# PAMRec/PAMRec

Measured on NVIDIA B200. Metric: train samples/sec, higher is better.
Workload: dtype f32

## Files before the change

pamrec_b200/csrc/api.cu:

```cuda
#include <cmath>
#include <cstdarg>
#include <cstdio>
#include <cstdlib>
#include <string>
#include <vector>

#include "comm.h"
#include "head2.h"
#include "kernels.h"
#include "layout.h"

using namespace pamrec;

struct Xchg {
  std::vector<int64_t> soff, scnt, roff, rcnt;
  int64_t n_send = 0, n_recv = 0;
};

struct PamrecHandle_ {
  PamrecConfig cfg;
  Layout L;
  PamrecBuffers buf;
  bool bound = false;
  int debug = 0;
  std::string err;
  int64_t launches = 0;
  Prof prof;
  BnSet bn[BN_COUNT];
  std::vector<int> h_seg_id, h_seg_tab;
  Comm comm;
  int* h_counts = nullptr;
  Xchg xc[3];
  bool xc_users = false;
  bool sharded() const { return cfg.table_mode == PAMREC_TABLES_SHARDED; }
  bool sibling() const { return cfg.model_kind != PAMREC_MODEL_PAMREC; }
  bool replicated() const { return cfg.table_mode == PAMREC_TABLES_REPLICATED && cfg.world_size > 1; }
  cudaStream_t side = nullptr;
  cudaEvent_t ev_side[16] = {};
  cudaEvent_t ev_join = nullptr, ev_plan = nullptr, ev_bucket = nullptr;
  int ev_next = 0;
  const void* plan_for = nullptr;
  int plan_rows = -1;
  void* mbox = nullptr;
  void* mbox_peer[kP2PMaxWorld] = {};
  bool mbox_open = false;
  unsigned* head_bar = nullptr;
  bool head_trace = false;
  unsigned long long* head_trace_cta = nullptr;
  uint32_t coop_epoch = 0;
  Head2 head2;
  int head2_grid = 0;
  bool use_head2() const { return head2_grid > 0 && (cfg.world_size == 1 || mbox_open); }
  uint32_t* mbox_err() const { return static_cast<uint32_t*>(mbox); }
  int64_t xr_dense() const { return (L.dense_numel + 63) / 64 * 64; }
  int64_t xr_floats() const { return xr_dense() + (replicated() ? sp2_rep_floats(cfg.n_items, cfg.n_cates, cfg.n_users) : 0); }
  char* xr_region(int p) const { return static_cast<char*>(mbox_peer[p]) + p2p_xr_offset(cfg.world_size); }
  bool use_xr() const { return mbox_open && cfg.world_size > 1; }
  uint32_t xr_epoch = 0;
  float* rep_grad_in() const { return use_xr() ? xr_xbuf(xr_region(cfg.rank)) + xr_dense() : wf("rep.grad"); }
  float* rep_grad_out() const {
    return use_xr() ? xr_xbuf(xr_region(cfg.rank)) + p2p_xr_cap(cfg.world_size, xr_floats()) + xr_dense() : wf("rep.grad");
  }
  ~PamrecHandle_() {
    if (h_counts) cudaFreeHost(h_counts);
    for (int p = 0; p < kP2PMaxWorld; ++p)
      if (mbox_peer[p] && mbox_peer[p] != mbox) cudaIpcCloseMemHandle(mbox_peer[p]);
    if (mbox) cudaFree(mbox);
    if (head_bar) cudaFree(head_bar);
    if (head_trace_cta) cudaFree(head_trace_cta);
    for (auto e : ev_side) if (e) cudaEventDestroy(e);
    if (ev_join) cudaEventDestroy(ev_join);
    if (ev_plan) cudaEventDestroy(ev_plan);
    if (ev_bucket) cudaEventDestroy(ev_bucket);
    if (side) cudaStreamDestroy(side);
  }
  template <typename F>
  void fork(cudaStream_t main, F fn) {
    cudaEvent_t e = ev_side[ev_next];
    ev_next = (ev_next + 1) % 16;
    cudaEventRecord(e, main);
    cudaStreamWaitEvent(side, e, 0);
    fn(side);
  }
  void join(cudaStream_t main) {
    cudaEventRecord(ev_join, side);
    cudaStreamWaitEvent(main, ev_join, 0);
  }

  float* P(int64_t off) const { return buf.dense_param + off; }
  float* G(int64_t off) const { return buf.dense_grad + off; }
  template <typename T>
  T* ws(const std::string& name) const { return reinterpret_cast<T*>(static_cast<char*>(buf.workspace) + L.ws_off(name)); }
  float* wf(const std::string& name) const { return ws<float>(name); }
  int* wi(const std::string& name) const { return ws<int>(name); }
  double* wd(const std::string& name) const { return ws<double>(name); }
};

struct ProfBind {
  PamrecHandle h; int64_t l0; Prof* prev;
  explicit ProfBind(PamrecHandle hh) : h(hh), l0(hh->prof.launches), prev(g_prof) { g_prof = &hh->prof; }
  ~ProfBind() { h->launches = h->prof.launches - l0; g_prof = prev; }
};

static int fail(PamrecHandle h, const char* fmt, ...) {
  char buf[512];
  va_list ap;
  va_start(ap, fmt);
  vsnprintf(buf, sizeof buf, fmt, ap);
  va_end(ap);
  if (h) h->err = buf;
  return -1;
}
static int check_cuda(PamrecHandle h, const char* where) {
  cudaError_t e = cudaGetLastError();
  if (e != cudaSuccess) return fail(h, "%s: %s", where, cudaGetErrorString(e));
  return 0;
}

extern "C" {

const char* pamrec_version(void) { return "pamrec_b200 0.1 (sm_100a)"; }

int pamrec_abi_sizes(int64_t out[6]) {
  if (!out) return -1;
  out[0] = sizeof(PamrecConfig); out[1] = sizeof(PamrecBatch); out[2] = sizeof(PamrecBuffers);
  out[3] = sizeof(PamrecTensorInfo); out[4] = sizeof(PamrecLines); out[5] = sizeof(PamrecVocab);
  return 0;
}

int pamrec_create(const PamrecConfig* cfg, PamrecHandle* out) {
  if (!cfg || !out) return -1;
  *out = nullptr;
  if (cfg->n_users < 1 || cfg->n_items < 1 || cfg->n_cates < 1) return -2;
  if (cfg->max_seq_len < 1 || cfg->max_seq_len > PAMREC_MAX_T) return -3;
  if (cfg->max_batch < 1) return -4;
  const int world = cfg->world_size < 1 ? 1 : cfg->world_size;
  if (world > 64 || cfg->rank < 0 || cfg->rank >= world) return -5;
  if (cfg->table_mode != PAMREC_TABLES_LOCAL && cfg->table_mode != PAMREC_TABLES_SHARDED && cfg->table_mode != PAMREC_TABLES_REPLICATED) return -6;
  if (world > 1 && cfg->table_mode == PAMREC_TABLES_LOCAL) return -6;
  if (cfg->table_mode != PAMREC_TABLES_SHARDED && (int64_t)cfg->n_items + cfg->n_cates + cfg->n_users >= ((int64_t)1 << 31)) return -7;
  if (cfg->loss_kind != PAMREC_LOSS_XENT && cfg->loss_kind != PAMREC_LOSS_SOFTMAX) return -8;
  if (cfg->loss_kind == PAMREC_LOSS_SOFTMAX) {
    const int g = cfg->softmax_group < 1 ? 1 : cfg->softmax_group;
    if (g > 1024 || (world > 1 && PAMREC_GROUP % g != 0)) return -8;
  }
  {
    int64_t big = cfg->n_items > cfg->n_users ? cfg->n_items : cfg->n_users;
    if (cfg->n_cates > big) big = cfg->n_cates;
    if (((big + world - 1) / world) * world >= ((int64_t)1 << 31)) return -7;
  }
  if (cfg->model_kind < PAMREC_MODEL_PAMREC || cfg->model_kind > PAMREC_MODEL_SASREC) return -9;
  if (cfg->model_kind != PAMREC_MODEL_PAMREC && (world != 1 || cfg->table_mode != PAMREC_TABLES_LOCAL || cfg->loss_kind != PAMREC_LOSS_XENT))
    return -9;
  const int di = cfg->item_dim ? cfg->item_dim : PAMREC_ITEM_DIM, dc = cfg->cate_dim ? cfg->cate_dim : PAMREC_CATE_DIM;
  const int du = cfg->user_dim ? cfg->user_dim : PAMREC_USER_DIM;
  if (!((di == 16 && dc == 4) || (di == 32 && dc == 8)) || !(du == 16 || du == 20 || du == 40)) return -10;
  if (cfg->model_kind == PAMREC_MODEL_PAMREC && (di != PAMREC_ITEM_DIM || dc != PAMREC_CATE_DIM || du != PAMREC_USER_DIM)) return -10;
  PamrecHandle h = new PamrecHandle_();
  h->cfg = *cfg;
  h->cfg.world_size = world;
  h->cfg.item_dim = di; h->cfg.cate_dim = dc; h->cfg.user_dim = du;
  if (h->cfg.softmax_group < 1) h->cfg.softmax_group = 1;
  h->L.build(h->cfg);
  const int n_seg = (int)h->L.dense.size();
  h->h_seg_id.assign((size_t)h->L.dense_numel, 0);
  h->h_seg_tab.assign((size_t)n_seg * 4, 0);
  for (int s = 0; s < n_seg; ++s) {
    const TensorDesc& t = h->L.dense[s];
    h->h_seg_tab[4 * s] = (int)t.offset;
    h->h_seg_tab[4 * s + 1] = (int)t.numel;
    h->h_seg_tab[4 * s + 2] = t.flags;
    for (int64_t i = 0; i < t.numel; ++i) h->h_seg_id[(size_t)(t.offset + i)] = s;
  }
  *out = h;
  return 0;
}

int pamrec_destroy(PamrecHandle h) {
  delete h;
  return 0;
}
const char* pamrec_last_error(PamrecHandle h) { return h ? h->err.c_str() : "null handle"; }
int64_t pamrec_dense_numel(PamrecHandle h) { return h ? h->L.dense_numel : -1; }
int64_t pamrec_bn_numel(PamrecHandle h) { return h ? h->L.bn_numel : -1; }
size_t pamrec_workspace_bytes(PamrecHandle h) { return h ? h->L.ws_bytes : 0; }
int64_t pamrec_last_launch_count(PamrecHandle h) { return h ? h->launches : -1; }
int64_t pamrec_shard_rows(PamrecHandle h, int64_t vocab_rows) { return h ? h->L.rows_of(vocab_rows) : -1; }

int pamrec_comm_unique_id(const char* nccl_path, char id_out[PAMREC_COMM_ID_BYTES]) {
  std::string err;
  if (Comm::unique_id(nccl_path, id_out, &err)) { fprintf(stderr, "pamrec_comm_unique_id: %s\n", err.c_str()); return -1; }
  return 0;
}
int pamrec_comm_init(PamrecHandle h, const char* nccl_path, const char id[PAMREC_COMM_ID_BYTES]) {
  if (!h || !id) return -1;
  if (h->comm.init(nccl_path, id, h->cfg.world_size, h->cfg.rank)) { h->err = "comm_init: " + h->comm.err; return -1; }
  return 0;
}
int pamrec_comm_mailbox_create(PamrecHandle h, char handle_out[PAMREC_IPC_HANDLE_BYTES]) {
  if (!h || !handle_out) return -1;
  static_assert(sizeof(cudaIpcMemHandle_t) == PAMREC_IPC_HANDLE_BYTES, "cudaIpcMemHandle_t is 64 bytes");
  if (h->cfg.world_size > kP2PMaxWorld) return fail(h, "mailboxes support at most %d ranks", kP2PMaxWorld);
  if (!h->mbox) {
    const size_t bytes = p2p_mailbox_bytes(h->cfg.world_size, h->xr_floats());
    if (cudaMalloc(&h->mbox, bytes) != cudaSuccess) return check_cuda(h, "mailbox alloc");
    cudaMemset(h->mbox, 0, bytes);
    cudaDeviceSynchronize();
  }
  cudaIpcMemHandle_t ih;
  if (cudaIpcGetMemHandle(&ih, h->mbox) != cudaSuccess) return check_cuda(h, "cudaIpcGetMemHandle");
  memcpy(handle_out, &ih, sizeof ih);
  return 0;
}
int pamrec_comm_mailbox_open(PamrecHandle h, const char* handles) {
  if (!h || !handles || !h->mbox) return -1;
  for (int p = 0; p < h->cfg.world_size; ++p) {
    if (p == h->cfg.rank) { h->mbox_peer[p] = h->mbox; continue; }
    cudaIpcMemHandle_t ih;
    memcpy(&ih, handles + (size_t)p * PAMREC_IPC_HANDLE_BYTES, sizeof ih);
    void* ptr = nullptr;
    if (cudaIpcOpenMemHandle(&ptr, ih, cudaIpcMemLazyEnablePeerAccess) != cudaSuccess) return check_cuda(h, "cudaIpcOpenMemHandle");
    h->mbox_peer[p] = ptr;
  }
  h->mbox_open = true;
  return 0;
}
int pamrec_comm_destroy(PamrecHandle h) {
  if (!h) return -1;
  h->comm.destroy();
  return 0;
}

static const std::vector<TensorDesc>* pool_of(PamrecHandle h, int pool) {
  if (!h) return nullptr;
  if (pool == PAMREC_POOL_DENSE) return &h->L.dense;
  if (pool == PAMREC_POOL_BN) return &h->L.bn;
  if (pool == PAMREC_POOL_WORKSPACE) return &h->L.ws;
  return nullptr;
}
int pamrec_tensor_count(PamrecHandle h, int pool) {
  auto* v = pool_of(h, pool);
  return v ? (int)v->size() : -1;
}
int pamrec_tensor_info(PamrecHandle h, int pool, int index, PamrecTensorInfo* out) {
  auto* v = pool_of(h, pool);
  if (!v || !out || index < 0 || index >= (int)v->size()) return -1;
  const TensorDesc& t = (*v)[index];
  memset(out, 0, sizeof *out);
  snprintf(out->name, sizeof out->name, "%s", t.name.c_str());
  out->pool = t.pool; out->dtype = t.dtype; out->flags = t.flags;
  out->offset = t.offset; out->numel = t.numel; out->ndim = t.ndim;
  for (int i = 0; i < 4; ++i) out->shape[i] = t.shape[i];
  return 0;
}

static BnSet make_bn(PamrecHandle h, int id, const char* name) {
  const BnOff& o = h->L.bnoff[id];
  BnSet s;
  s.C = o.C;
  s.gamma = h->P(o.gamma); s.beta = h->P(o.beta);
  s.dgamma = h->G(o.gamma); s.dbeta = h->G(o.beta);
  s.mmean = h->buf.bn_moving + o.mm; s.mvar = h->buf.bn_moving + o.mv;
  std::string p = std::string("bn.") + name;
  s.sums = h->wd(p + ".sums"); s.stat = h->wf(p + ".stat"); s.bsums = h->wd("bn.bsums") + h->L.bn_bsums_off[id];
  return s;
}

static int build_head(PamrecHandle h, cudaStream_t st);
static HeadDyn head_dyn(PamrecHandle h, const PamrecBatch* b, bool training, int slot0);

int pamrec_bind(PamrecHandle h, const PamrecBuffers* bufs, void* stream) {
  if (!h || !bufs) return -1;
  cudaStream_t st = (cudaStream_t)stream;
  if (bufs->workspace_bytes < h->L.ws_bytes) return fail(h, "workspace too small: %zu < %zu", bufs->workspace_bytes, h->L.ws_bytes);
  if (!bufs->dense_param || !bufs->dense_grad || !bufs->dense_m || !bufs->dense_v || !bufs->bn_moving || !bufs->item_w ||
      !bufs->cate_w || !bufs->ulong_w || !bufs->ushort_w || !bufs->workspace)
    return fail(h, "null buffer");
  int ndev = 0;
  if (cudaGetDeviceCount(&ndev) != cudaSuccess || ndev == 0) { cudaGetLastError(); return fail(h, "no CUDA device: the CUDA path is the only path"); }
  h->buf = *bufs;
  if (init_encoder_kernels(h->cfg.max_seq_len)) return check_cuda(h, "shared-memory opt-in of the encoder kernels");
  if (h->cfg.model_kind == PAMREC_MODEL_SASREC && init_sas_kernels(h->cfg.max_seq_len))
    return check_cuda(h, "shared-memory opt-in of the SASRec attention kernels");
  if (init_attn_mma_kernels(h->cfg.max_seq_len)) return check_cuda(h, "shared-memory opt-in of the MMA attention kernels");
  if (!h->side) {
    if (cudaStreamCreateWithFlags(&h->side, cudaStreamNonBlocking) != cudaSuccess) return fail(h, "cannot create the side stream");
    for (auto& e : h->ev_side) cudaEventCreateWithFlags(&e, cudaEventDisableTiming);
    cudaEventCreateWithFlags(&h->ev_join, cudaEventDisableTiming);
    cudaEventCreateWithFlags(&h->ev_plan, cudaEventDisableTiming);
    cudaEventCreateWithFlags(&h->ev_bucket, cudaEventDisableTiming);
  }
  static const char* names[BN_COUNT] = {"s0", "s1", "e0", "g0", "e1", "g1", "t0", "t1"};
  for (int i = 0; i < BN_COUNT; ++i) h->bn[i] = make_bn(h, i, names[i]);
  size_t need = sparse_temp_bytes(h->L.cub_keys);
  if (!h->sharded()) { const size_t n2 = sp2_temp_bytes(h->L.cub_keys); need = n2 > need ? n2 : need; }
  size_t have = (size_t)h->L.ws[h->L.ws_index["cub_temp"]].numel;
  if (need > have) return fail(h, "cub temp storage: need %zu have %zu", need, have);
  cudaMemsetAsync(h->buf.workspace, 0, h->L.ws_bytes, st);
  if (h->sharded() || h->sibling()) {
    cudaMemsetAsync(h->wi("sp.item.slot"), 0xFF, (size_t)h->L.rows_of(h->cfg.n_items) * 4, st);
    cudaMemsetAsync(h->wi("sp.cate.slot"), 0xFF, (size_t)h->L.rows_of(h->cfg.n_cates) * 4, st);
    if (h->cfg.model_kind != PAMREC_MODEL_SASREC)
      cudaMemsetAsync(h->wi("sp.user.slot"), 0xFF, (size_t)h->L.rows_of(h->cfg.n_users) * 4, st);
  } else {
    cudaMemsetAsync(h->wi("sp2.slot"), 0xFF, ((size_t)h->cfg.n_items + h->cfg.n_cates + h->cfg.n_users) * 4, st);
  }
  if (h->sharded() && !h->h_counts &&
      cudaMallocHost(&h->h_counts, sizeof(int) * (8 * (size_t)h->cfg.world_size + 4)) != cudaSuccess)
    return fail(h, "cudaMallocHost for the exchange counts failed");
  cudaMemcpyAsync(h->wi("seg_id"), h->h_seg_id.data(), h->h_seg_id.size() * 4, cudaMemcpyHostToDevice, st);
  cudaMemcpyAsync(h->wi("seg_tab"), h->h_seg_tab.data(), h->h_seg_tab.size() * 4, cudaMemcpyHostToDevice, st);
  if (h->sibling()) h->head2_grid = 0;
  else if (int rc = build_head(h, st)) return rc;
  cudaStreamSynchronize(st);
  h->bound = true;
  return check_cuda(h, "bind");
}

static int check_batch(PamrecHandle h, const PamrecBatch* b, bool training) {
  if (!h) return -1;
  if (!h->bound) return fail(h, "pamrec_bind has not been called");
  if (!b) return fail(h, "null batch");
  if (b->batch == 0 && (h->sharded() || h->cfg.world_size > 1)) return 0;
  if (b->batch < 1 || b->batch > h->cfg.max_batch) return fail(h, "batch %d outside [1, %d]", b->batch, h->cfg.max_batch);
  if (h->sibling()) {
    if (!b->satisfied_item_history || !b->satisfied_cate_history || !b->satisfied_mask || !b->item_history || !b->item_cate_history ||
        !b->mask || !b->items || !b->cates)
      return fail(h, "null batch field (the sibling models also read satisfied_item_history / satisfied_cate_history / satisfied_mask)");
    const bool sas = h->cfg.model_kind == PAMREC_MODEL_SASREC;
    if (training && (!b->labels_satisfied || (!sas && (!b->users || !b->labels_play)))) return fail(h, "null label field");
    return 0;
  }
  if (training && b->batch % PAMREC_GROUP != 0)
    return fail(h, "training batch %d is not a multiple of %d (pamrec.py:73-75)", b->batch, PAMREC_GROUP);
  if (training && h->cfg.loss_kind == PAMREC_LOSS_SOFTMAX && b->batch % h->cfg.softmax_group != 0)
    return fail(h, "training batch %d is not a multiple of the softmax group %d (base_model.py:224-225)", b->batch, h->cfg.softmax_group);
  if (!b->item_history || !b->item_cate_history || !b->item_loop_times_history || !b->mask || !b->items || !b->cates)
    return fail(h, "null batch field");
  if (training && (!b->users || !b->labels_satisfied || !b->labels_play || !b->plays)) return fail(h, "null label field");
  return 0;
}

static Sp2 make_sp2(PamrecHandle h, const PamrecBatch* b) {
  Sp2 s;
  memset(&s, 0, sizeof s);
  const PamrecConfig& c = h->cfg;
  s.item_hist = b->item_history; s.cate_hist = b->item_cate_history; s.items = b->items; s.cates = b->cates; s.users = b->users;
  s.B = b->batch; s.N = (int64_t)b->batch * c.max_seq_len;
  s.n_items = c.n_items; s.n_cates = c.n_cates; s.n_users = c.n_users;
  s.keys = h->wi("sp2.keys"); s.idx = h->wi("sp2.idx"); s.skeys = h->wi("sp2.skeys"); s.sidx = h->wi("sp2.sidx"); s.uidx = h->wi("sp2.uidx");
  s.ukeys[0] = h->wi("sp.item.ukeys"); s.ukeys[1] = h->wi("sp.cate.ukeys"); s.ukeys[2] = h->wi("sp.user.ukeys");
  s.nuniq = h->wi("sp.nuniq"); s.meta = h->wi("sp2.meta");
  s.accum[0] = h->wf("sp.item.accum"); s.accum[1] = h->wf("sp.cate.accum");
  s.dflag[0] = h->wi("sp2.dflag"); s.dflag[1] = s.dflag[0] + h->L.cub_keys_table;
  s.l2sq = h->wd("sp2.l2sq"); s.undedup = h->wd("sp_normsq");
  s.w[0] = h->buf.item_w; s.m[0] = h->buf.item_m; s.v[0] = h->buf.item_v;
  s.w[1] = h->buf.cate_w; s.m[1] = h->buf.cate_m; s.v[1] = h->buf.cate_v;
  s.w[2] = h->buf.ulong_w; s.m[2] = h->buf.ulong_m; s.v[2] = h->buf.ulong_v;
  s.w[3] = h->buf.ushort_w; s.m[3] = h->buf.ushort_m; s.v[3] = h->buf.ushort_v;
  s.dX0 = h->wf("g_a"); s.dT = h->wf("d_tgt_total");
  if (h->replicated()) { s.mode = SP2_DENSE; s.rep_grad = h->rep_grad_in(); }
  else if (c.sparse_adam_mode == PAMREC_ADAM_LAZY) s.mode = SP2_FUSED;
  else { s.mode = SP2_COMPACT; s.slot = h->wi("sp2.slot"); }
  return s;
}
static AdamP make_adam(PamrecHandle h, float lr_t) {
  const PamrecConfig& c = h->cfg;
  AdamP a;
  a.lr = lr_t; a.b1 = c.beta1; a.b2 = c.beta2; a.eps = c.epsilon; a.l2 = c.embed_l2; a.clip = c.max_grad_norm; a.is_clip = c.is_clip_norm;
  a.lr_dev = nullptr;
  return a;
}

static const char* const kShardName[3] = {"item", "cate", "user"};
static const ShardDim& shard_dim(PamrecHandle h, int t) { return t == 0 ? h->L.sh_item : (t == 1 ? h->L.sh_cate : h->L.sh_user); }

static SparseTable req_table(PamrecHandle h, int t) {
  SparseTable s;
  memset(&s, 0, sizeof s);
  const ShardDim& d = shard_dim(h, t);
  std::string p = std::string("sp.") + kShardName[t] + ".";
  s.keys = h->wi(p + "keys"); s.idx = h->wi(p + "idx"); s.skeys = h->wi(p + "skeys"); s.sidx = h->wi(p + "sidx");
  s.uidx = h->wi(p + "uidx"); s.ukeys = h->wi(p + "ukeys");
  s.width = d.width; s.n_rows = d.rps * h->cfg.world_size;
  s.accum = d.width ? h->wf(p + "accum") : nullptr;
  s.nuniq = h->wi("sp.nuniq") + t;
  s.normsq = h->wd("sp_normsq") + t;
  return s;
}
static SparseTable own_table(PamrecHandle h, int t, bool user_short = false) {
  SparseTable s;
  memset(&s, 0, sizeof s);
  const ShardDim& d = shard_dim(h, t);
  std::string q = std::string("so.") + kShardName[t] + ".";
  s.keys = h->wi(q + "keys"); s.idx = h->wi(q + "idx"); s.skeys = h->wi(q + "skeys"); s.sidx = h->wi(q + "sidx");
  s.uidx = h->wi(q + "uidx"); s.ukeys = h->wi(q + "ukeys");
  s.slot = h->wi(std::string("sp.") + kShardName[t] + ".slot");
  s.n_rows = d.rps;
  s.nuniq = h->wi("sp.nuniq") + 4 + t;
  double* ns = h->wd("sp_normsq");
  if (t == 0) { s.width = kI; s.w = h->buf.item_w; s.m = h->buf.item_m; s.v = h->buf.item_v; s.accum = h->wf(q + "accum"); s.normsq = ns; }
  else if (t == 1) { s.width = kC; s.w = h->buf.cate_w; s.m = h->buf.cate_m; s.v = h->buf.cate_v; s.accum = h->wf(q + "accum"); s.normsq = ns + 1; }
  else if (!user_short) { s.width = PAMREC_USER_DIM; s.w = h->buf.ulong_w; s.m = h->buf.ulong_m; s.v = h->buf.ulong_v; s.normsq = ns + 2; }
  else { s.width = PAMREC_USER_DIM; s.w = h->buf.ushort_w; s.m = h->buf.ushort_m; s.v = h->buf.ushort_v; s.normsq = ns + 3; }
  return s;
}

static int shard_exchange_fwd(PamrecHandle h, const PamrecBatch* b, bool training, cudaStream_t st) {
  const int W = h->cfg.world_size, B = b->batch, T = h->cfg.max_seq_len;
  const int64_t N = (int64_t)B * T;
  void* tmp = h->ws<char>("cub_temp");
  const size_t tmp_bytes = (size_t)h->L.ws[h->L.ws_index.at("cub_temp")].numel;
  int* cs = h->wi("sh.counts_send");
  int* cr = h->wi("sh.counts_recv");
  cudaMemsetAsync(cs, 0, sizeof(int) * 4 * W, st);
  const int nt = training ? 3 : 2;
  h->xc_users = training;
  for (int t = 0; t < nt; ++t) {
    const ShardDim& d = shard_dim(h, t);
    SparseTable req = req_table(h, t);
    const int* hist = t == 0 ? b->item_history : (t == 1 ? b->item_cate_history : b->users);
    const int* tgt = t == 0 ? b->items : (t == 1 ? b->cates : nullptr);
    const int64_t n_hist = t < 2 ? N : B, n_tgt = t < 2 ? B : 0;
    if (launch_sparse_plan(req, hist, tgt, n_hist, n_tgt, W, d.rps, d.rps * W, false, tmp, tmp_bytes, st))
      return fail(h, "cub sort failed");
    std::string p = std::string("sh.") + kShardName[t] + ".";
    launch_shard_route(req, n_hist + n_tgt, W, d.rps, h->wi(p + "off"), cs, t, h->wi(p + "send_ids"), h->wi(p + "inv"), st);
  }
  {
    PAMREC_PROF("xchg_counts", 1, st);
    if (h->comm.all_to_all(cs, cr, 4, COMM_I32, st)) return fail(h, "nccl: %s", h->comm.err.c_str());
    cudaMemcpyAsync(h->h_counts, cs, sizeof(int) * 4 * W, cudaMemcpyDeviceToHost, st);
    cudaMemcpyAsync(h->h_counts + 4 * W, cr, sizeof(int) * 4 * W, cudaMemcpyDeviceToHost, st);
    h->h_counts[8 * W] = 0;
    if (h->mbox_open) cudaMemcpyAsync(h->h_counts + 8 * W, h->mbox_err(), sizeof(int), cudaMemcpyDeviceToHost, st);
    if (cudaStreamSynchronize(st) != cudaSuccess) return check_cuda(h, "exchange counts");
    if (h->h_counts[8 * W]) return fail(h, "peer mailbox all-reduce timed out at sync point %d (a rank left the step?)", h->h_counts[8 * W] - 1);
  }
  for (int t = 0; t < 3; ++t) {
    Xchg& x = h->xc[t];
    x.soff.assign(W, 0); x.scnt.assign(W, 0); x.roff.assign(W, 0); x.rcnt.assign(W, 0);
    int64_t so = 0, ro = 0;
    for (int p = 0; p < W; ++p) {
      x.scnt[p] = t < nt ? h->h_counts[4 * p + t] : 0;
      x.rcnt[p] = t < nt ? h->h_counts[4 * W + 4 * p + t] : 0;
      x.soff[p] = so; so += x.scnt[p];
      x.roff[p] = ro; ro += x.rcnt[p];
    }
    x.n_send = so; x.n_recv = ro;
    if (ro > shard_dim(h, t).cap_recv) return fail(h, "exchange overflow on table %s: %lld rows", kShardName[t], (long long)ro);
  }
  {
    PAMREC_PROF("xchg_ids", 1, st);
    int xrc = h->comm.group_start();
    for (int t = 0; t < nt && !xrc; ++t) {
      const Xchg& x = h->xc[t];
      std::string p = std::string("sh.") + kShardName[t] + ".";
      xrc |= h->comm.all_to_all_v(h->wi(p + "send_ids"), x.soff.data(), x.scnt.data(), h->wi(p + "recv_ids"), x.roff.data(),
                                  x.rcnt.data(), 1, COMM_I32, st);
    }
    xrc |= h->comm.group_end();
    if (xrc) return fail(h, "nccl: %s", h->comm.err.c_str());
  }
  if (training) {
    int prc = 0;
    h->fork(st, [&](cudaStream_t s2) {
      for (int t = 0; t < 3; ++t) {
        SparseTable own = own_table(h, t);
        std::string p = std::string("sh.") + kShardName[t] + ".";
        prc |= launch_sparse_plan(own, h->wi(p + "recv_ids"), nullptr, h->xc[t].n_recv, 0, 1, 0, own.n_rows, true, tmp, tmp_bytes, s2);
      }
      cudaEventRecord(h->ev_plan, s2);
    });
    if (prc) return fail(h, "cub sort failed");
  }
  launch_serve_rows(h->buf.item_w, h->wi("sh.item.recv_ids"), h->xc[0].n_recv, kI, h->wf("sh.item.xrows"), st);
  launch_serve_rows(h->buf.cate_w, h->wi("sh.cate.recv_ids"), h->xc[1].n_recv, kC, h->wf("sh.cate.xrows"), st);
  {
    PAMREC_PROF("xchg_rows", 1, st);
    int xrc = h->comm.group_start();
    for (int t = 0; t < 2 && !xrc; ++t) {
      const Xchg& x = h->xc[t];
      std::string p = std::string("sh.") + kShardName[t] + ".";
      xrc |= h->comm.all_to_all_v(h->wf(p + "xrows"), x.roff.data(), x.rcnt.data(), h->wf(p + "rows"), x.soff.data(),
                                  x.scnt.data(), shard_dim(h, t).width, COMM_F32, st);
    }
    xrc |= h->comm.group_end();
    if (xrc) return fail(h, "nccl: %s", h->comm.err.c_str());
  }
  return 0;
}

static int embed_forward(PamrecHandle h, const PamrecBatch* b, bool training, float* x0, cudaStream_t st) {
  const int B = b->batch, T = h->cfg.max_seq_len;
  if (!h->sharded()) {
    launch_embed_fwd(b->item_history, b->item_cate_history, b->items, b->cates, h->buf.item_w, h->buf.cate_w, h->P(h->L.pos), x0,
                     h->wf("tgt"), B, T, st);
    return 0;
  }
  if (int rc = shard_exchange_fwd(h, b, training, st)) return rc;
  const int64_t N = (int64_t)B * T;
  const int* ii = h->wi("sh.item.inv");
  const int* ci = h->wi("sh.cate.inv");
  launch_embed_fwd(ii, ci, ii + N, ci + N, h->wf("sh.item.rows"), h->wf("sh.cate.rows"), h->P(h->L.pos), x0, h->wf("tgt"), B, T, st);
  return 0;
}

int pamrec_gather_fwd(PamrecHandle h, const PamrecBatch* b, float* x0_out, void* stream) {
  if (int rc = check_batch(h, b, false)) return rc;
  if (h->sibling()) return fail(h, "pamrec_gather_fwd is PAMRec's fused gather; the sibling models gather inside pamrec_forward");
  ProfBind _pb(h);
  cudaStream_t st = (cudaStream_t)stream;
  if (int rc = embed_forward(h, b, false, x0_out ? x0_out : h->wf("x0"), st)) return rc;
  return check_cuda(h, "gather_fwd");
}

static DenseP dense_p(const float* X, int ldx, int M, int groups, int K, int N, const float* W, int ws, const float* bias,
                      int bs, float* Z, int ldz) {
  DenseP p;
  memset(&p, 0, sizeof p);
  p.X = X; p.ldx = ldx; p.M = M; p.n_groups = groups; p.K = K; p.N = N;
  p.W = W; p.w_stride = ws; p.bias = bias; p.b_stride = bs; p.Z = Z; p.ldz = ldz;
  return p;
}
static void set_in_bn(DenseP& p, const BnSet& s) { p.in_stat = s.stat; p.in_gamma = s.gamma; p.in_beta = s.beta; }
static void set_in_bn_dw(DenseDwP& p, const BnSet& s) { p.in_stat = s.stat; p.in_gamma = s.gamma; p.in_beta = s.beta; }

static int sib_forward(PamrecHandle h, const PamrecBatch* b, int training, float* pred_out, cudaStream_t st);
static int sib_backward(PamrecHandle h, const PamrecBatch* b, cudaStream_t st);
static int sib_apply(PamrecHandle h, const PamrecBatch* b, int64_t step, cudaStream_t st);
static int sas_forward(PamrecHandle h, const PamrecBatch* b, int training, float* pred_out, cudaStream_t st);
static int sas_backward(PamrecHandle h, const PamrecBatch* b, cudaStream_t st);
static int head_forward(PamrecHandle h, const PamrecBatch* b, bool training, float* pred_out, cudaStream_t st);

int pamrec_forward(PamrecHandle h, const PamrecBatch* b, int training, float* pred_out, void* stream) {
  if (int rc = check_batch(h, b, training != 0)) return rc;
  ProfBind _pb(h);
  cudaStream_t st = (cudaStream_t)stream;
  if (h->cfg.model_kind == PAMREC_MODEL_SASREC) return sas_forward(h, b, training, pred_out, st);
  if (h->sibling()) return sib_forward(h, b, training, pred_out, st);
  const Layout& L = h->L;
  const int B = b->batch, T = h->cfg.max_seq_len, N = B * T;
  float* x0 = h->wf("x0");
  int* ctl = h->wi("bucket_ctl");
  const bool bucket_aside = !h->sharded();
  if (bucket_aside) {
    h->fork(st, [&](cudaStream_t s2) {
      launch_bucket_plan(b->item_loop_times_history, N, h->wi("bucket"), h->wi("perm"), ctl, h->wi("tile_bucket"), h->wi("tile_begin"),
                         h->wi("tile_count"), s2);
      cudaEventRecord(h->ev_bucket, s2);
    });
  }
  if (int rc = embed_forward(h, b, training != 0, x0, st)) return rc;
  if (training && !h->sharded() && B > 0) {
    int prc = 0;
    h->fork(st, [&](cudaStream_t s2) {
      prc |= launch_sp2_plan(make_sp2(h, b), h->ws<char>("cub_temp"), (size_t)L.ws[L.ws_index.at("cub_temp")].numel, s2);
      cudaEventRecord(h->ev_plan, s2);
    });
    if (prc) return fail(h, "cub sort failed");
    h->plan_for = b->item_history; h->plan_rows = B;
  }
  if (bucket_aside) cudaStreamWaitEvent(st, h->ev_bucket, 0);
  else launch_bucket_plan(b->item_loop_times_history, N, h->wi("bucket"), h->wi("perm"), ctl, h->wi("tile_bucket"),
                          h->wi("tile_begin"), h->wi("tile_count"), st);
  const int max_tiles = N / kTokTile + kNB + 1;
  const float* xin = x0;
  for (int k = 0; k < 2; ++k) {
    const BlockOff& o = L.blk[k];
    std::string p = "blk" + std::to_string(k) + ".";
    launch_proj_fwd(xin, h->wi("perm"), ctl, h->wi("tile_bucket"), h->wi("tile_begin"), h->wi("tile_count"), max_tiles,
                    h->P(o.wq), h->P(o.wk), h->P(o.wv), h->P(o.ln_a_beta), h->P(o.ln_a_gamma), h->wf(p + "qin"), h->wf(p + "Q"),
                    h->wf(p + "K"), h->wf(p + "V"), st);
    if (T <= 128)
      launch_attn_fwd_mma(h->wf(p + "Q"), h->wf(p + "K"), h->wf(p + "V"), h->wf(p + "qin"), b->mask, h->wf(p + "y"), h->wf(p + "pv"), h->wf(p + "ml"), B, T, st);
    else
      launch_attn_fwd(h->wf(p + "Q"), h->wf(p + "K"), h->wf(p + "V"), h->wf(p + "qin"), b->mask, h->wf(p + "y"), h->wf(p + "pv"), h->wf(p + "ml"), B, T, st);
    float* hdbg = (training && (h->debug & PAMREC_DEBUG_SAVE_FFN_HIDDEN)) ? h->wf(k == 0 ? "d_Q" : "d_K") : nullptr;
    launch_ffn_fwd(h->wf(p + "y"), h->P(o.w1), h->P(o.b1), h->P(o.w2), h->P(o.b2), h->P(o.ln_b_beta), h->P(o.ln_b_gamma),
                   h->wf(p + "out"), hdbg, N, st);
    xin = h->wf(p + "out");
  }
  if (h->use_head2()) {
    HeadDyn d = head_dyn(h, b, training != 0, 0);
    d.pred = pred_out;
    if (launch_head2_fwd(h->head2, d, h->head2_grid, training ? "head_fwd" : "head_score", st)) return check_cuda(h, "cooperative head launch");
  } else if (int rc = head_forward(h, b, training != 0, pred_out, st)) {
    return rc;
  }
  return check_cuda(h, "forward");
}

static int head_forward(PamrecHandle h, const PamrecBatch* b, bool training, float* pred_out, cudaStream_t st) {
  const Layout& L = h->L;
  const int B = b->batch, T = h->cfg.max_seq_len, N = B * T;
  const int W = h->cfg.world_size;
  const int Bg = b->global_batch > 0 ? b->global_batch : B * W;
  const double cntN = (double)Bg * T, cntB = (double)Bg;
  int crc = 0;
  auto sync_finalize = [&](std::initializer_list<int> ids, double cnt, bool with_scalars) {
    if (!training) return;
    if (W > 1 && !crc) {
      PAMREC_PROF("allreduce_bn_fwd", 1, st);
      crc |= h->comm.group_start();
      for (int id : ids) crc |= h->comm.all_reduce(h->bn[id].sums, 2 * (int64_t)h->bn[id].C, COMM_F64, st);
      if (with_scalars) crc |= h->comm.all_reduce(h->wd("dp.scalars"), 8, COMM_F64, st);
      crc |= h->comm.group_end();
    }
    for (int id : ids) launch_bn_finalize(h->bn[id], cnt, st);
  };
  if (training && W > 1) {
    cudaMemsetAsync(h->wd("dp.scalars"), 0, 8 * sizeof(double), st);
    launch_count_valid_groups(b->plays, B, h->wd("dp.scalars"), st);
  }
  const float* H = h->wf("blk1.out");
  BnSet* bn = h->bn;
  if (!training) {
    for (int i = 0; i < BN_COUNT; ++i) launch_bn_eval_stat(bn[i], st);
  }
  {
    DenseP p = dense_p(H, kD, N, 1, kD, 20, h->P(L.score.w0), 0, h->P(L.score.b0), 0, h->wf("z1"), 20);
    p.out_sums = training ? bn[BN_S0].sums : nullptr;
    launch_dense_fwd(p, st);
    sync_finalize({BN_S0}, cntN, true);
    DenseP q = dense_p(h->wf("z1"), 20, N, 1, 20, 1, h->P(L.score.w1), 0, h->P(L.score.b1), 0, h->wf("z2"), 1);
    set_in_bn(q, bn[BN_S0]);
    q.out_sums = training ? bn[BN_S1].sums : nullptr;
    launch_dense_fwd(q, st);
    sync_finalize({BN_S1}, cntN, false);
  }
  launch_pool_fwd(H, h->wf("z2"), bn[BN_S1], b->mask, h->wf("new_long"), B, T, st);
  {
    DenseP e0 = dense_p(h->wf("new_long"), kD, B, 5, kD, 100, h->P(L.expert.w0), 4000, h->P(L.expert.b0), 100, h->wf("ze0"), 500);
    for (int g = 0; g < 5; ++g) { e0.x_off[g] = 0; e0.z_off[g] = g * 100; }
    e0.out_sums = training ? bn[BN_E0].sums : nullptr;
    launch_dense_fwd(e0, st);
    DenseP g0 = dense_p(h->wf("new_long"), kD, B, 2, kD, 64, h->P(L.gate.w0), 2560, h->P(L.gate.b0), 64, h->wf("zg0"), 128);
    for (int g = 0; g < 2; ++g) { g0.x_off[g] = 0; g0.z_off[g] = g * 64; }
    g0.out_sums = training ? bn[BN_G0].sums : nullptr;
    launch_dense_fwd(g0, st);
    sync_finalize({BN_E0, BN_G0}, cntB, false);
    DenseP e1 = dense_p(h->wf("ze0"), 500, B, 5, 100, 64, h->P(L.expert.w1), 6400, h->P(L.expert.b1), 64, h->wf("ze1"), 320);
    for (int g = 0; g < 5; ++g) { e1.x_off[g] = g * 100; e1.z_off[g] = g * 64; }
    set_in_bn(e1, bn[BN_E0]);
    e1.out_sums = training ? bn[BN_E1].sums : nullptr;
    launch_dense_fwd(e1, st);
    DenseP g1 = dense_p(h->wf("zg0"), 128, B, 2, 64, 5, h->P(L.gate.w1), 320, h->P(L.gate.b1), 5, h->wf("zg1"), 10);
    for (int g = 0; g < 2; ++g) { g1.x_off[g] = g * 64; g1.z_off[g] = g * 5; }
    set_in_bn(g1, bn[BN_G0]);
    g1.out_sums = training ? bn[BN_G1].sums : nullptr;
    launch_dense_fwd(g1, st);
    sync_finalize({BN_E1, BN_G1}, cntB, false);
  }
  launch_combine_fwd(h->wf("ze1"), h->wf("zg1"), bn[BN_E1], bn[BN_G1], h->wf("tgt"), h->wf("u"), B, st);
  {
    DenseP t0 = dense_p(h->wf("u"), 168, B, 3, 84, 100, h->P(L.tower.w0), 8400, h->P(L.tower.b0), 100, h->wf("zt0"), 300);
    t0.x_off[0] = 0; t0.x_off[1] = 84; t0.x_off[2] = 0;
    for (int g = 0; g < 3; ++g) t0.z_off[g] = g * 100;
    t0.out_sums = training ? bn[BN_T0].sums : nullptr;
    launch_dense_fwd(t0, st);
    sync_finalize({BN_T0}, cntB, false);
    DenseP t1 = dense_p(h->wf("zt0"), 300, B, 3, 100, 64, h->P(L.tower.w1), 6400, h->P(L.tower.b1), 64, h->wf("zt1"), 192);
    for (int g = 0; g < 3; ++g) { t1.x_off[g] = g * 100; t1.z_off[g] = g * 64; }
    set_in_bn(t1, bn[BN_T0]);
    t1.out_sums = training ? bn[BN_T1].sums : nullptr;
    launch_dense_fwd(t1, st);
    sync_finalize({BN_T1}, cntB, false);
    DenseP to = dense_p(h->wf("zt1"), 192, B, 3, 64, 1, h->P(L.tower.wout), 64, h->P(L.tower.bout), 1, h->wf("logits"), 3);
    for (int g = 0; g < 3; ++g) { to.x_off[g] = g * 64; to.z_off[g] = g; }
    set_in_bn(to, bn[BN_T1]);
    launch_dense_fwd(to, st);
  }
  if (pred_out) launch_sigmoid_col0(h->wf("logits"), pred_out, B, st);
  if (crc) return fail(h, "nccl: %s", h->comm.err.c_str());
  return 0;
}

static DenseDwP dw_p(const float* X, int ldx, int M, int groups, int K, int N, const float* dZ, int lddz, float* dW, int ws,
                     float* db, int bs) {
  DenseDwP p;
  memset(&p, 0, sizeof p);
  p.X = X; p.ldx = ldx; p.M = M; p.n_groups = groups; p.K = K; p.N = N; p.dZ = dZ; p.lddz = lddz;
  p.dW = dW; p.w_stride = ws; p.db = db; p.b_stride = bs;
  return p;
}
static DenseDxP dx_p(const float* dZ, int lddz, int M, int K, const float* Wbase, float* dX, int lddx, int accumulate) {
  DenseDxP p;
  memset(&p, 0, sizeof p);
  p.dZ = dZ; p.lddz = lddz; p.M = M; p.K = K; p.Wbase = Wbase; p.dX = dX; p.lddx = lddx; p.accumulate = accumulate;
  return p;
}
static void dx_add(DenseDxP& p, int slice, int out_off, int dz_off, int64_t w_off, int N) {
  if (slice >= p.n_slices) { p.n_slices = slice + 1; p.out_off[slice] = out_off; p.n_contrib[slice] = 0; }
  int c = p.n_contrib[slice]++;
  p.dz_off[slice][c] = dz_off; p.w_off[slice][c] = w_off; p.Ncon[slice][c] = N;
}

static HeadDyn head_dyn(PamrecHandle h, const PamrecBatch* b, bool training, int slot0) {
  HeadDyn d;
  memset(&d, 0, sizeof d);
  const int W = h->cfg.world_size;
  d.B = b->batch; d.T = h->cfg.max_seq_len; d.training = training ? 1 : 0; d.world = W; d.rank = h->cfg.rank;
  d.Bg = b->global_batch > 0 ? b->global_batch : b->batch * W;
  d.cntN = (double)d.Bg * d.T; d.cntB = (double)d.Bg;
  d.mask = b->mask; d.y_sat = b->labels_satisfied; d.y_play = b->labels_play; d.plays = b->plays;
  d.fuzhu_w = h->cfg.fuzhu_weight; d.order_w = h->cfg.order_weight;
  d.sm_group = h->cfg.loss_kind == PAMREC_LOSS_SOFTMAX ? h->cfg.softmax_group : 0;
  d.bar = h->head_bar;
  d.trace = h->head_trace ? reinterpret_cast<unsigned long long*>(h->head_bar + 64) + (slot0 ? 32 : 0) : nullptr;
  d.trace_cta = (h->head_trace && h->head_trace_cta) ? h->head_trace_cta + (slot0 ? 16 * 256 : 0) : nullptr;
  if (W > 1) {
    for (int p = 0; p < W; ++p) d.peer_ll[p] = reinterpret_cast<uint4*>(static_cast<char*>(h->mbox_peer[p]) + p2p_ll_offset());
    d.p2p_epoch = ++h->coop_epoch; d.p2p_slot0 = slot0; d.p2p_err = h->mbox_err();
  }
  return d;
}

static int build_head(PamrecHandle h, cudaStream_t st) {
  h->head2_grid = 0;
  if (getenv("PAMREC_HEAD_LEGACY") != nullptr) return 0;
  if (h->cfg.world_size > kP2PMaxWorld) return 0;
  const Layout& L = h->L;
  Head2& H = h->head2;
  memset(&H, 0, sizeof H);
  H.H = h->wf("blk1.out"); H.tgt = h->wf("tgt");
  H.s_w0 = h->P(L.score.w0); H.s_b0 = h->P(L.score.b0); H.s_w1 = h->P(L.score.w1); H.s_b1 = h->P(L.score.b1);
  H.e_w0 = h->P(L.expert.w0); H.e_b0 = h->P(L.expert.b0); H.e_w1 = h->P(L.expert.w1); H.e_b1 = h->P(L.expert.b1);
  H.g_w0 = h->P(L.gate.w0); H.g_b0 = h->P(L.gate.b0); H.g_w1 = h->P(L.gate.w1); H.g_b1 = h->P(L.gate.b1);
  H.t_w0 = h->P(L.tower.w0); H.t_b0 = h->P(L.tower.b0); H.t_w1 = h->P(L.tower.w1); H.t_b1 = h->P(L.tower.b1);
  H.t_wo = h->P(L.tower.wout); H.t_bo = h->P(L.tower.bout);
  H.ds_w0 = h->G(L.score.w0); H.ds_b0 = h->G(L.score.b0); H.ds_w1 = h->G(L.score.w1); H.ds_b1 = h->G(L.score.b1);
  H.de_w0 = h->G(L.expert.w0); H.de_b0 = h->G(L.expert.b0); H.de_w1 = h->G(L.expert.w1); H.de_b1 = h->G(L.expert.b1);
  H.dg_w0 = h->G(L.gate.w0); H.dg_b0 = h->G(L.gate.b0); H.dg_w1 = h->G(L.gate.w1); H.dg_b1 = h->G(L.gate.b1);
  H.dt_w0 = h->G(L.tower.w0); H.dt_b0 = h->G(L.tower.b0); H.dt_w1 = h->G(L.tower.w1); H.dt_b1 = h->G(L.tower.b1);
  H.dt_wo = h->G(L.tower.wout); H.dt_bo = h->G(L.tower.bout);
  H.wT = h->wf("head.wT");
  static_assert(kHead2Groups == 8, "layout.h: bn.gsums / bn.gbsums hold 8 copies");
  for (int i = 0; i < BN_COUNT; ++i) {
    H.bn[i] = h->bn[i];
    H.gsums[i] = h->wd("bn.gsums") + (size_t)kHead2Groups * L.bn_bsums_off[i];
    H.gbsums[i] = h->wd("bn.gbsums") + (size_t)kHead2Groups * L.bn_bsums_off[i];
  }
  H.z1 = h->wf("z1"); H.z2 = h->wf("z2"); H.aw = h->wf("pool.aw"); H.new_long = h->wf("new_long");
  H.ze0 = h->wf("ze0"); H.zg0 = h->wf("zg0"); H.ze1 = h->wf("ze1"); H.zg1 = h->wf("zg1"); H.u = h->wf("u");
  H.zt0 = h->wf("zt0"); H.zt1 = h->wf("zt1"); H.logits = h->wf("logits");
  H.d_logits = h->wf("d_logits"); H.d_t1 = h->wf("d_t1"); H.d_t0 = h->wf("d_t0"); H.d_e1 = h->wf("d_e1"); H.d_g1 = h->wf("d_g1");
  H.d_e0 = h->wf("d_e0"); H.d_g0 = h->wf("d_g0"); H.d_new_long = h->wf("d_new_long"); H.d_tgt = h->wf("d_tgt");
  H.d_z2 = h->wf("d_z2"); H.g_a = h->wf("g_a");
  H.loss_acc = h->wd("loss_acc"); H.dp_scalars = h->wd("dp.scalars");
  const int g2 = head2_grid();
  if (g2 <= 0) { cudaGetLastError(); return 0; }
  if (!h->head_bar) {
    if (cudaMalloc(&h->head_bar, 256 + 2 * 32 * 8) != cudaSuccess) return check_cuda(h, "head barrier alloc");
    cudaMemsetAsync(h->head_bar, 0, 256 + 2 * 32 * 8, st);
  }
  h->head2_grid = g2;
  return check_cuda(h, "head2");
}

static int head_backward(PamrecHandle h, const PamrecBatch* b, cudaStream_t st) {
  const Layout& L = h->L;
  const int B = b->batch, T = h->cfg.max_seq_len, N = B * T;
  const int W = h->cfg.world_size;
  const int Bg = b->global_batch > 0 ? b->global_batch : B * W;
  const double cntN = (double)Bg * T, cntB = (double)Bg;
  const float gs = 1.0f / (float)W;
  BnSet* bn = h->bn;
  int crc = 0;
  const float* Pb = h->buf.dense_param;
  launch_loss(h->wf("logits"), b->labels_satisfied, b->labels_play, b->plays, h->wf("d_logits"), h->wd("loss_acc"), B, Bg,
              W > 1 ? h->wd("dp.scalars") : nullptr, h->cfg.fuzhu_weight, h->cfg.order_weight,
              h->cfg.loss_kind == PAMREC_LOSS_SOFTMAX ? h->cfg.softmax_group : 0, st);
  cudaMemsetAsync(h->wd("bn.bsums"), 0, (size_t)L.ws[L.ws_index.at("bn.bsums")].numel * sizeof(double), st);
  auto sync_bsums = [&](std::initializer_list<int> ids) {
    if (W == 1 || crc) return;
    PAMREC_PROF("allreduce_bn_bwd", 1, st);
    crc |= h->comm.group_start();
    for (int id : ids) crc |= h->comm.all_reduce(bn[id].bsums, 2 * (int64_t)bn[id].C, COMM_F64, st);
    crc |= h->comm.group_end();
  };
  auto grad_of = [&](int id, const float* Z, double cnt) {
    BnGrad g; g.Z = Z; g.stat = bn[id].stat; g.gamma = bn[id].gamma; g.beta = bn[id].beta; g.bsums = bn[id].bsums; g.count = cnt;
    return g;
  };
  auto out_of = [&](int id, const float* Z) {
    BnGradOut o; o.Z = Z; o.stat = bn[id].stat; o.gamma = bn[id].gamma; o.beta = bn[id].beta; o.bsums = bn[id].bsums;
    return o;
  };
  auto dw_bn = [&](DenseDwP& w, int id, const float* Z, double cnt) {
    w.g = grad_of(id, Z, cnt); w.g_dgamma = bn[id].dgamma; w.g_dbeta = bn[id].dbeta; w.g_C = bn[id].C; w.g_scale = gs;
  };
  {
    DenseDwP w = dw_p(h->wf("zt1"), 192, B, 3, 64, 1, h->wf("d_logits"), 3, h->G(L.tower.wout), 64, h->G(L.tower.bout), 1);
    for (int g = 0; g < 3; ++g) { w.x_off[g] = g * 64; w.z_off[g] = g; }
    set_in_bn_dw(w, bn[BN_T1]);
    h->fork(st, [&](cudaStream_t s2) { launch_dense_dw(w, s2); });
    DenseDxP x = dx_p(h->wf("d_logits"), 3, B, 64, Pb, h->wf("d_t1"), 192, 0);
    for (int g = 0; g < 3; ++g) dx_add(x, g, g * 64, g, L.tower.wout + g * 64, 1);
    x.o = out_of(BN_T1, h->wf("zt1"));
    launch_dense_dx(x, st);
    sync_bsums({BN_T1});
    DenseDwP w1 = dw_p(h->wf("zt0"), 300, B, 3, 100, 64, h->wf("d_t1"), 192, h->G(L.tower.w1), 6400, h->G(L.tower.b1), 64);
    for (int g = 0; g < 3; ++g) { w1.x_off[g] = g * 100; w1.z_off[g] = g * 64; }
    set_in_bn_dw(w1, bn[BN_T0]);
    dw_bn(w1, BN_T1, h->wf("zt1"), cntB);
    h->fork(st, [&](cudaStream_t s2) { launch_dense_dw(w1, s2); });
    DenseDxP x1 = dx_p(h->wf("d_t1"), 192, B, 100, Pb, h->wf("d_t0"), 300, 0);
    for (int g = 0; g < 3; ++g) dx_add(x1, g, g * 100, g * 64, L.tower.w1 + (int64_t)g * 6400, 64);
    x1.g = grad_of(BN_T1, h->wf("zt1"), cntB);
    x1.o = out_of(BN_T0, h->wf("zt0"));
    launch_dense_dx(x1, st);
    sync_bsums({BN_T0});
    DenseDwP w0 = dw_p(h->wf("u"), 168, B, 3, 84, 100, h->wf("d_t0"), 300, h->G(L.tower.w0), 8400, h->G(L.tower.b0), 100);
    w0.x_off[0] = 0; w0.x_off[1] = 84; w0.x_off[2] = 0;
    for (int g = 0; g < 3; ++g) w0.z_off[g] = g * 100;
    dw_bn(w0, BN_T0, h->wf("zt0"), cntB);
    h->fork(st, [&](cudaStream_t s2) { launch_dense_dw(w0, s2); });
    DenseDxP x0 = dx_p(h->wf("d_t0"), 300, B, 84, Pb, h->wf("d_u"), 168, 0);
    dx_add(x0, 0, 0, 0, L.tower.w0, 100);
    dx_add(x0, 0, 0, 200, L.tower.w0 + 2 * 8400, 100);
    dx_add(x0, 1, 84, 100, L.tower.w0 + 8400, 100);
    x0.g = grad_of(BN_T0, h->wf("zt0"), cntB);
    launch_dense_dx(x0, st);
  }
  launch_combine_bwd(h->wf("ze1"), h->wf("zg1"), bn[BN_E1], bn[BN_G1], h->wf("d_u"), h->wf("d_e1"), h->wf("d_g1"),
                     h->wf("d_tgt"), B, st);
  {
    launch_bn_bwd_stats(bn[BN_E1], h->wf("d_e1"), h->wf("ze1"), B, st);
    launch_bn_bwd_stats(bn[BN_G1], h->wf("d_g1"), h->wf("zg1"), B, st);
    sync_bsums({BN_E1, BN_G1});
    DenseDwP we = dw_p(h->wf("ze0"), 500, B, 5, 100, 64, h->wf("d_e1"), 320, h->G(L.expert.w1), 6400, h->G(L.expert.b1), 64);
    for (int g = 0; g < 5; ++g) { we.x_off[g] = g * 100; we.z_off[g] = g * 64; }
    set_in_bn_dw(we, bn[BN_E0]);
    dw_bn(we, BN_E1, h->wf("ze1"), cntB);
    h->fork(st, [&](cudaStream_t s2) { launch_dense_dw(we, s2); });
    DenseDxP xe = dx_p(h->wf("d_e1"), 320, B, 100, Pb, h->wf("d_e0"), 500, 0);
    for (int g = 0; g < 5; ++g) dx_add(xe, g, g * 100, g * 64, L.expert.w1 + (int64_t)g * 6400, 64);
    xe.g = grad_of(BN_E1, h->wf("ze1"), cntB);
    xe.o = out_of(BN_E0, h->wf("ze0"));
    launch_dense_dx(xe, st);
    DenseDwP wg = dw_p(h->wf("zg0"), 128, B, 2, 64, 5, h->wf("d_g1"), 10, h->G(L.gate.w1), 320, h->G(L.gate.b1), 5);
    for (int g = 0; g < 2; ++g) { wg.x_off[g] = g * 64; wg.z_off[g] = g * 5; }
    set_in_bn_dw(wg, bn[BN_G0]);
    dw_bn(wg, BN_G1, h->wf("zg1"), cntB);
    h->fork(st, [&](cudaStream_t s2) { launch_dense_dw(wg, s2); });
    DenseDxP xg = dx_p(h->wf("d_g1"), 10, B, 64, Pb, h->wf("d_g0"), 128, 0);
    for (int g = 0; g < 2; ++g) dx_add(xg, g, g * 64, g * 5, L.gate.w1 + (int64_t)g * 320, 5);
    xg.g = grad_of(BN_G1, h->wf("zg1"), cntB);
    xg.o = out_of(BN_G0, h->wf("zg0"));
    launch_dense_dx(xg, st);
    sync_bsums({BN_E0, BN_G0});
    DenseDwP we0 = dw_p(h->wf("new_long"), kD, B, 5, kD, 100, h->wf("d_e0"), 500, h->G(L.expert.w0), 4000, h->G(L.expert.b0), 100);
    for (int g = 0; g < 5; ++g) { we0.x_off[g] = 0; we0.z_off[g] = g * 100; }
    dw_bn(we0, BN_E0, h->wf("ze0"), cntB);
    h->fork(st, [&](cudaStream_t s2) { launch_dense_dw(we0, s2); });
    DenseDwP wg0 = dw_p(h->wf("new_long"), kD, B, 2, kD, 64, h->wf("d_g0"), 128, h->G(L.gate.w0), 2560, h->G(L.gate.b0), 64);
    for (int g = 0; g < 2; ++g) { wg0.x_off[g] = 0; wg0.z_off[g] = g * 64; }
    dw_bn(wg0, BN_G0, h->wf("zg0"), cntB);
    h->fork(st, [&](cudaStream_t s2) { launch_dense_dw(wg0, s2); });
    DenseDxP xe0 = dx_p(h->wf("d_e0"), 500, B, kD, Pb, h->wf("d_new_long"), kD, 0);
    for (int g = 0; g < 5; ++g) dx_add(xe0, 0, 0, g * 100, L.expert.w0 + (int64_t)g * 4000, 100);
    xe0.g = grad_of(BN_E0, h->wf("ze0"), cntB);
    launch_dense_dx(xe0, st);
    DenseDxP xg0 = dx_p(h->wf("d_g0"), 128, B, kD, Pb, h->wf("d_new_long"), kD, 1);
    for (int g = 0; g < 2; ++g) dx_add(xg0, 0, 0, g * 64, L.gate.w0 + (int64_t)g * 2560, 64);
    xg0.g = grad_of(BN_G0, h->wf("zg0"), cntB);
    launch_dense_dx(xg0, st);
  }
  const float* H = h->wf("blk1.out");
  float* g_a = h->wf("g_a");
  launch_pool_bwd(H, h->wf("z2"), bn[BN_S1], b->mask, h->wf("d_new_long"), h->wf("d_z2"), g_a, B, T, st);
  launch_bn_bwd_stats(bn[BN_S1], h->wf("d_z2"), h->wf("z2"), N, st);
  sync_bsums({BN_S1});
  DenseDwP w1 = dw_p(h->wf("z1"), 20, N, 1, 20, 1, h->wf("d_z2"), 1, h->G(L.score.w1), 0, h->G(L.score.b1), 0);
  set_in_bn_dw(w1, bn[BN_S0]);
  dw_bn(w1, BN_S1, h->wf("z2"), cntN);
  h->fork(st, [&](cudaStream_t s2) { launch_dense_dw(w1, s2); });
  DenseDxP x1 = dx_p(h->wf("d_z2"), 1, N, 20, Pb, h->wf("d_a1"), 20, 0);
  dx_add(x1, 0, 0, 0, L.score.w1, 1);
  x1.g = grad_of(BN_S1, h->wf("z2"), cntN);
  x1.o = out_of(BN_S0, h->wf("z1"));
  launch_dense_dx(x1, st);
  sync_bsums({BN_S0});
  DenseDwP w0 = dw_p(H, kD, N, 1, kD, 20, h->wf("d_a1"), 20, h->G(L.score.w0), 0, h->G(L.score.b0), 0);
  dw_bn(w0, BN_S0, h->wf("z1"), cntN);
  h->fork(st, [&](cudaStream_t s2) { launch_dense_dw(w0, s2); });
  DenseDxP x0 = dx_p(h->wf("d_a1"), 20, N, kD, Pb, g_a, kD, 1);
  dx_add(x0, 0, 0, 0, L.score.w0, 20);
  x0.g = grad_of(BN_S0, h->wf("z1"), cntN);
  launch_dense_dx(x0, st);
  return crc;
}

int pamrec_backward(PamrecHandle h, const PamrecBatch* b, void* stream) {
  if (int rc = check_batch(h, b, true)) return rc;
  ProfBind _pb(h);
  cudaStream_t st = (cudaStream_t)stream;
  if (h->cfg.model_kind == PAMREC_MODEL_SASREC) return sas_backward(h, b, st);
  if (h->sibling()) return sib_backward(h, b, st);
  const Layout& L = h->L;
  const int B = b->batch, T = h->cfg.max_seq_len, N = B * T;
  int crc = 0;
  cudaMemsetAsync(h->buf.dense_grad, 0, (size_t)L.dense_numel * 4, st);
  cudaMemsetAsync(h->wd("loss_acc"), 0, 8 * sizeof(double), st);
  cudaMemsetAsync(h->wd("sp_normsq"), 0, 8 * sizeof(double), st);
  if (h->use_head2()) {
    cudaMemsetAsync(h->wd("bn.bsums"), 0, (size_t)L.ws[L.ws_index.at("bn.bsums")].numel * sizeof(double), st);
    HeadDyn d = head_dyn(h, b, true, 12);
    if (launch_head2_bwd(h->head2, d, h->head2_grid, st)) return check_cuda(h, "cooperative head launch");
    h->fork(st, [&](cudaStream_t s2) { launch_head2_dw(h->head2, B, s2); });
  } else {
    crc = head_backward(h, b, st);
  }
  float* g_a = h->wf("g_a");
  float* g_b = h->wf("g_b");
  const int max_tiles = N / kTokTile + kNB + 1;
  int* ctl = h->wi("bucket_ctl");
  for (int k = 1; k >= 0; --k) {
    const BlockOff& o = L.blk[k];
    std::string p = "blk" + std::to_string(k) + ".";
    const float* xin = k == 0 ? h->wf("x0") : h->wf("blk0.out");
    float* gout = k == 1 ? g_a : g_b;
    float* gin = k == 1 ? g_b : g_a;
    float* dQ = h->wf(k == 1 ? "blk1.d_Q" : "d_Q");
    float* dK = h->wf(k == 1 ? "blk1.d_K" : "d_K");
    float* dV = h->wf(k == 1 ? "blk1.d_V" : "d_V");
    float* dout = k == 1 ? h->wf("blk1.d_out") : gout;
    EncDwArgs dw{h->wf(p + "qin"), xin, dQ, dK, dV, h->wi("perm"), ctl, h->wf(p + "y"), h->P(o.ln_b_beta), h->P(o.ln_b_gamma),
                 h->wf(p + "h"), h->wf(p + "dhr"), dout, h->G(o.wq), h->G(o.wk), h->G(o.wv), h->G(o.w1), h->G(o.b1), h->G(o.w2),
                 h->G(o.b2), N, true};
    launch_ffn_bwd(h->wf(p + "y"), gout, h->P(o.w1), h->P(o.b1), h->P(o.w2), h->P(o.ln_b_beta), h->P(o.ln_b_gamma), h->wf("d_y"),
                   h->wf(p + "h"), h->wf(p + "dhr"), k == 1 ? dout : nullptr, h->G(o.ln_b_beta), h->G(o.ln_b_gamma), N, st);
    h->fork(st, [&](cudaStream_t s2) { launch_enc_dw(dw, s2); });
    if (T <= 128)
      launch_attn_bwd_mma(h->wf(p + "Q"), h->wf(p + "K"), h->wf(p + "V"), h->wf("d_y"), h->wf(p + "pv"), h->wf(p + "ml"),
                          b->mask, dQ, dK, dV, B, T, st);
    else
      launch_attn_bwd(h->wf(p + "Q"), h->wf(p + "K"), h->wf(p + "V"), h->wf("d_y"), h->wf(p + "pv"), h->wf(p + "ml"),
                      b->mask, dQ, dK, dV, B, T, st);
    dw.ffn = false;
    h->fork(st, [&](cudaStream_t s2) { launch_enc_dw(dw, s2); });
    launch_proj_bwd(xin, h->wf("d_y"), dQ, dK, dV, h->wi("perm"), ctl, h->wi("tile_bucket"), h->wi("tile_begin"), h->wi("tile_count"),
                    max_tiles, h->P(o.wq), h->P(o.wk), h->P(o.wv), h->P(o.ln_a_beta), h->P(o.ln_a_gamma), gin, h->G(o.ln_a_beta),
                    h->G(o.ln_a_gamma), st);
  }
  launch_embed_bwd_reduce(g_a, h->wf("d_tgt"), h->wf("d_tgt_total"), h->G(L.pos), h->wd("sp_normsq") + 4,
                          h->sharded() ? nullptr : h->wd("sp_normsq"), B, T, st);
  h->join(st);
  if (crc) return fail(h, "nccl: %s", h->comm.err.c_str());
  return check_cuda(h, "backward");
}

static void peer_allreduce_grads(PamrecHandle h, cudaStream_t st) {
  XrArgs a;
  memset(&a, 0, sizeof a);
  const int W = h->cfg.world_size;
  for (int p = 0; p < W; ++p) a.peer[p] = h->xr_region(p);
  a.world = W; a.rank = h->cfg.rank; a.epoch = ++h->xr_epoch;
  a.cap = p2p_xr_cap(W, h->xr_floats());
  a.dense_grad = h->buf.dense_grad; a.n_dense = h->L.dense_numel;
  a.scalars[0] = h->wd("sp_normsq"); a.n_scalars[0] = 8;
  a.scalars[1] = h->wd("loss_acc"); a.n_scalars[1] = 4;
  a.counter = reinterpret_cast<unsigned*>(h->xr_region(h->cfg.rank) + 128);
  a.err = h->mbox_err();
  launch_xr_allreduce(a, h->buf.dense_grad, st);
}

int pamrec_apply_gradients(PamrecHandle h, const PamrecBatch* b, int64_t step, void* stream) {
  if (int rc = check_batch(h, b, true)) return rc;
  ProfBind _pb(h);
  if (h->sibling()) return sib_apply(h, b, step, (cudaStream_t)stream);
  if (step < 0) return fail(h, "step must be >= 1 (or 0: advance the device step counter)");
  if (step == 0 && (h->sharded() || h->cfg.world_size > 1)) return fail(h, "the device step counter (step = 0) needs one GPU with whole tables");
  cudaStream_t st = (cudaStream_t)stream;
  const Layout& L = h->L;
  const PamrecConfig& c = h->cfg;
  const int B = b->batch, T = c.max_seq_len;
  const int64_t N = (int64_t)B * T;
  const double b1 = c.beta1, b2 = c.beta2;
  const double tstep = step > 0 ? (double)step : 1.0;
  const float lr_t = (float)((double)c.learning_rate * std::sqrt(1.0 - std::pow(b2, tstep)) / (1.0 - std::pow(b1, tstep)));
  const float* lr_dev = nullptr;
  if (!h->sharded()) {
    launch_adam_step(step, h->wd("adam.step"), c.learning_rate, c.beta1, c.beta2, h->wf("adam.lr"), st);
    lr_dev = h->wf("adam.lr");
  }
  double* reg = h->wd("loss_acc") + 3;
  void* tmp = h->ws<char>("cub_temp");
  size_t tmp_bytes = (size_t)L.ws[L.ws_index.at("cub_temp")].numel;
  bool dense_aside = false;
  const float* dX0 = h->wf("g_a");
  const float* dT = h->wf("d_tgt_total");
  if (h->sharded()) {
    Comm& cm = h->comm;
    int crc = 0;
    if (!h->xc_users) return fail(h, "apply_gradients needs pamrec_forward(training=1) on the same batch");
    for (int t = 0; t < 2; ++t) {
      SparseTable req = req_table(h, t);
      const int col = t == 0 ? 0 : kI;
      launch_sparse_segreduce(req, N + B, N, dX0, kD, col, dT, kE, col, req.normsq, st);
    }
    {
      PAMREC_PROF("xchg_grads", 1, st);
      crc |= cm.group_start();
      for (int t = 0; t < 2; ++t) {
        const Xchg& x = h->xc[t];
        std::string p = std::string("sh.") + kShardName[t] + ".";
        crc |= cm.all_to_all_v(req_table(h, t).accum, x.soff.data(), x.scnt.data(), h->wf(p + "xrows"), x.roff.data(), x.rcnt.data(),
                               shard_dim(h, t).width, COMM_F32, st);
      }
      crc |= cm.group_end();
    }
    cudaStreamWaitEvent(st, h->ev_plan, 0);
    for (int t = 0; t < 3; ++t) {
      SparseTable own = own_table(h, t);
      const int64_t nr = h->xc[t].n_recv;
      std::string p = std::string("sh.") + kShardName[t] + ".";
      if (t < 2) launch_sparse_segreduce(own, nr, nr, h->wf(p + "xrows"), own.width, 0, nullptr, 0, 0, h->wd("sh.scratch"), st);
      launch_sparse_l2norm(own, nr, c.embed_l2, reg, st);
      if (t == 2) launch_sparse_l2norm(own_table(h, 2, true), nr, c.embed_l2, reg, st);
    }
    if (h->use_xr()) {
      peer_allreduce_grads(h, st);
    } else {
      PAMREC_PROF("allreduce_grads", 1, st);
      crc |= cm.group_start();
      crc |= cm.all_reduce(h->buf.dense_grad, L.dense_numel, COMM_F32, st);
      crc |= cm.all_reduce(h->wd("sp_normsq"), 8, COMM_F64, st);
      crc |= cm.all_reduce(h->wd("loss_acc"), 4, COMM_F64, st);
      crc |= cm.group_end();
    }
    if (crc) return fail(h, "nccl: %s", cm.err.c_str());
    for (int t = 0; t < 3; ++t) {
      SparseTable own = own_table(h, t);
      const int64_t nr = h->xc[t].n_recv;
      launch_sparse_adam(own, nr, c.sparse_adam_mode, c.embed_l2, lr_t, c.beta1, c.beta2, c.epsilon, c.max_grad_norm, c.is_clip_norm, st);
      if (t == 2)
        launch_sparse_adam(own_table(h, 2, true), nr, c.sparse_adam_mode, c.embed_l2, lr_t, c.beta1, c.beta2, c.epsilon,
                           c.max_grad_norm, c.is_clip_norm, st);
      launch_slot_reset(own, nr, st);
    }
  } else {
    if (c.world_size == 1) {
      dense_aside = true;
      h->fork(st, [&](cudaStream_t s2) {
        launch_dense_norm(h->buf.dense_param, h->buf.dense_grad, h->wi("seg_tab"), (int)L.dense.size(), c.layer_l2, h->wd("seg_normsq"),
                          h->wd("sp_normsq") + 4, reg, s2);
        launch_dense_adam(h->buf.dense_param, h->buf.dense_grad, h->buf.dense_m, h->buf.dense_v, h->wi("seg_id"), h->wi("seg_tab"),
                          h->wd("seg_normsq"), L.dense_numel, c.layer_l2, lr_t, lr_dev, c.beta1, c.beta2, c.epsilon, c.max_grad_norm,
                          c.is_clip_norm, s2);
      });
    }
    const bool planned = h->plan_for == b->item_history && h->plan_rows == B;
    h->plan_for = nullptr;
    const Sp2 s2 = make_sp2(h, b);
    AdamP ap = make_adam(h, lr_t);
    ap.lr_dev = lr_dev;
    if (planned) cudaStreamWaitEvent(st, h->ev_plan, 0);
    else if (launch_sp2_plan(s2, tmp, tmp_bytes, st)) return fail(h, "cub sort failed");
    launch_sp2_walk(s2, ap, st);
   
    if (h->replicated()) {
      Sp2 s3 = s2;
      if (h->use_xr()) {
        peer_allreduce_grads(h, st);
        s3.rep_grad = h->rep_grad_out();
      } else {
        Comm& cm = h->comm;
        int crc = 0;
        {
          PAMREC_PROF("allreduce_grads", 1, st);
          crc |= cm.group_start();
          crc |= cm.all_reduce(h->buf.dense_grad, L.dense_numel, COMM_F32, st);
          crc |= cm.all_reduce(s2.rep_grad, sp2_rep_floats(c.n_items, c.n_cates, c.n_users), COMM_F32, st);
          crc |= cm.all_reduce(h->wd("sp_normsq"), 8, COMM_F64, st);
          crc |= cm.all_reduce(h->wd("loss_acc"), 4, COMM_F64, st);
          crc |= cm.group_end();
        }
        if (crc) return fail(h, "nccl: %s", cm.err.c_str());
      }
      launch_sp2_rep_l2(s3, st);
      launch_sp2_adam_sweep(s3, ap, c.sparse_adam_mode == PAMREC_ADAM_LAZY ? 1 : 0, st);
     
    } else if (s2.mode == SP2_FUSED) {
      launch_sp2_lazy_finish(s2, ap, st);
    } else {
      launch_sp2_adam_sweep(s2, ap, 0, st);
    }
  }
  const int n_seg = (int)L.dense.size();
  if (dense_aside) {
    h->join(st);
  } else {
    launch_dense_norm(h->buf.dense_param, h->buf.dense_grad, h->wi("seg_tab"), n_seg, c.layer_l2, h->wd("seg_normsq"),
                      h->wd("sp_normsq") + 4, reg, st);
    launch_dense_adam(h->buf.dense_param, h->buf.dense_grad, h->buf.dense_m, h->buf.dense_v, h->wi("seg_id"), h->wi("seg_tab"),
                      h->wd("seg_normsq"), L.dense_numel, c.layer_l2, lr_t, lr_dev, c.beta1, c.beta2, c.epsilon, c.max_grad_norm,
                      c.is_clip_norm, st);
  }
  launch_finish_losses(h->wd("loss_acc"), h->wf("losses"), h->sharded() ? nullptr : h->wd("sp2.l2sq"), c.embed_l2, h->wd("sp_normsq"), st);
 
  return check_cuda(h, "apply_gradients");
}

#include "api_sibling.inl"

int pamrec_train_step(PamrecHandle h, const PamrecBatch* b, int64_t step, float* losses_out, void* stream) {
  if (!h) return -1;
  const int64_t l0 = h->prof.launches;
  if (int rc = pamrec_forward(h, b, 1, nullptr, stream)) return rc;
  if (int rc = pamrec_backward(h, b, stream)) return rc;
  if (int rc = pamrec_apply_gradients(h, b, step, stream)) return rc;
  if (losses_out)
    cudaMemcpyAsync(losses_out, h->wf("losses"), 5 * sizeof(float), cudaMemcpyDeviceToDevice, (cudaStream_t)stream);
  h->launches = h->prof.launches - l0;
  return check_cuda(h, "train_step");
}

int pamrec_comm_all_reduce(PamrecHandle h, void* dptr, int64_t count, int dtype, void* stream) {
  if (!h) return -1;
  CommType t = dtype == PAMREC_F64 ? COMM_F64 : (dtype == PAMREC_I32 ? COMM_I32 : COMM_F32);
  if (h->comm.all_reduce(dptr, count, t, (cudaStream_t)stream)) return fail(h, "nccl: %s", h->comm.err.c_str());
  return 0;
}

int pamrec_bench_gather(PamrecHandle h, const int32_t* item_ids, const int32_t* cate_ids, const int32_t* tgt_items,
                        const int32_t* tgt_cates, int64_t n_rows, int32_t T, float* out, void* stream) {
  if (!h || !h->bound) return fail(h, "not bound");
  if (h->sibling()) return fail(h, "bench_gather measures PAMRec's fused gather");
  if (T < 1 || T > h->cfg.max_seq_len) return fail(h, "T outside the position table");
  ProfBind _pb(h);
  launch_embed_fwd(item_ids, cate_ids, tgt_items, tgt_cates, h->buf.item_w, h->buf.cate_w, h->P(h->L.pos), out, nullptr, n_rows,
                   T, (cudaStream_t)stream);
  return check_cuda(h, "bench_gather");
}

int pamrec_bench_table_adam(PamrecHandle h, int64_t step, void* stream) {
  if (!h || !h->bound) return fail(h, "not bound");
  ProfBind _pb(h);
  const PamrecConfig& c = h->cfg;
  const double b1 = c.beta1, b2 = c.beta2;
  const float lr_t = (float)((double)c.learning_rate * std::sqrt(1.0 - std::pow(b2, (double)step)) / (1.0 - std::pow(b1, (double)step)));
  if (h->sharded() || h->sibling()) return fail(h, "bench_table_adam runs on PAMRec's whole tables");
  PamrecBatch nb;
  memset(&nb, 0, sizeof nb);
  Sp2 s2 = make_sp2(h, &nb);
  s2.mode = SP2_COMPACT; s2.slot = h->wi("sp2.slot");
  launch_sp2_adam_sweep(s2, make_adam(h, lr_t), 0, (cudaStream_t)stream);
  return check_cuda(h, "bench_table_adam");
}

int pamrec_set_debug(PamrecHandle h, int flags) {
  if (!h) return -1;
  h->debug = flags;
  h->head_trace = (flags & PAMREC_DEBUG_HEAD_TRACE) != 0;
  if (h->head_trace && !h->head_trace_cta && cudaMalloc(&h->head_trace_cta, 2 * 16 * 256 * 8) == cudaSuccess)
    cudaMemset(h->head_trace_cta, 0, 2 * 16 * 256 * 8);
  return 0;
}
int pamrec_head_trace_ctas(PamrecHandle h, int backward, uint64_t* out ) {
  if (!h || !out || !h->head_trace_cta) return -1;
  cudaDeviceSynchronize();
  if (cudaMemcpy(out, h->head_trace_cta + (backward ? 16 * 256 : 0), 16 * 256 * 8, cudaMemcpyDeviceToHost) != cudaSuccess) return check_cuda(h, "head trace");
  return 0;
}
int pamrec_head_trace(PamrecHandle h, int backward, uint64_t out[32]) {
  if (!h || !out || !h->head_bar) return -1;
  cudaDeviceSynchronize();
  if (cudaMemcpy(out, reinterpret_cast<unsigned long long*>(h->head_bar + 64) + (backward ? 32 : 0), 32 * 8, cudaMemcpyDeviceToHost) != cudaSuccess)
    return check_cuda(h, "head trace");
  return 0;
}
int pamrec_profile_enable(PamrecHandle h, int on) {
  if (!h) return -1;
  h->prof.on = on != 0;
  return 0;
}
int pamrec_profile_reset(PamrecHandle h) {
  if (!h) return -1;
  h->prof.reset();
  return 0;
}
int pamrec_profile_count(PamrecHandle h) {
  if (!h) return -1;
  h->prof.resolve();
  return (int)h->prof.names.size();
}
int pamrec_profile_get(PamrecHandle h, int index, char name[64], double* total_ms, int64_t* launches) {
  if (!h || index < 0 || index >= (int)h->prof.names.size()) return -1;
  snprintf(name, 64, "%s", h->prof.names[index].c_str());
  if (total_ms) *total_ms = h->prof.ms[index];
  if (launches) *launches = h->prof.cnt[index];
  return 0;
}

}
```

pamrec_b200/csrc/head2.h:

```cpp
#pragma once
#include "headcoop.h"
#include "layout.h"

namespace pamrec {

constexpr int kHead2Threads = 512;
constexpr int kHead2Groups = 8;
constexpr int kHead2WtFloats = 3 * 6400 + 3 * 8400 + 5 * 6400 + 2 * 320 + 628 * 40;

struct Head2 {
  const float* H;
  const float* tgt;
  const float *s_w0, *s_b0, *s_w1, *s_b1;
  const float *e_w0, *e_b0, *e_w1, *e_b1;
  const float *g_w0, *g_b0, *g_w1, *g_b1;
  const float *t_w0, *t_b0, *t_w1, *t_b1, *t_wo, *t_bo;
  float *ds_w0, *ds_b0, *ds_w1, *ds_b1, *de_w0, *de_b0, *de_w1, *de_b1, *dg_w0, *dg_b0, *dg_w1, *dg_b1;
  float *dt_w0, *dt_b0, *dt_w1, *dt_b1, *dt_wo, *dt_bo;
  float* wT;
  BnSet bn[BN_COUNT];
  double* gsums[BN_COUNT];
  double* gbsums[BN_COUNT];
  float *z1, *z2, *aw, *new_long, *ze0, *zg0, *ze1, *zg1, *u, *zt0, *zt1, *logits;
  float *d_logits, *d_t1, *d_t0, *d_e1, *d_g1, *d_e0, *d_g0, *d_new_long, *d_tgt, *d_z2, *g_a;
  double* loss_acc;
  double* dp_scalars;
};

int head2_grid();
int launch_head2_fwd(const Head2& h, const HeadDyn& d, int grid, const char* name, cudaStream_t st);
int launch_head2_bwd(const Head2& h, const HeadDyn& d, int grid, cudaStream_t st);
void launch_head2_dw(const Head2& h, int B, cudaStream_t st);

}
```

pamrec_b200/csrc/kernels_head2.cu:

```cuda
#include <cstdio>

#include "head2.h"

namespace pamrec {

namespace {

constexpr int kT2 = kHead2Threads;
constexpr int kRC = 8;
constexpr int kXS = 640;
constexpr int kWBuf = 32768;
constexpr int kSlots = 25;

__device__ __forceinline__ void st_release_u32(unsigned* p, unsigned v) { asm volatile("st.release.gpu.global.u32 [%0], %1;" ::"l"(p), "r"(v) : "memory"); }
__device__ __forceinline__ unsigned ld_relaxed_u32(const unsigned* p) {
  unsigned v;
  asm volatile("ld.relaxed.gpu.global.u32 %0, [%1];" : "=r"(v) : "l"(p) : "memory");
  return v;
}
__device__ __forceinline__ void fence_acq_rel_gpu() { asm volatile("fence.acq_rel.gpu;" ::: "memory"); }
__device__ __forceinline__ void st_flag_sys(uint32_t* p, uint32_t v) { asm volatile("st.release.sys.global.u32 [%0], %1;" ::"l"(p), "r"(v) : "memory"); }
__device__ __forceinline__ uint32_t ld_flag_sys_relaxed(const uint32_t* p) {
  uint32_t v;
  asm volatile("ld.relaxed.sys.global.u32 %0, [%1];" : "=r"(v) : "l"(p) : "memory");
  return v;
}
__device__ __forceinline__ void fence_acq_rel_sys() { asm volatile("fence.acq_rel.sys;" ::: "memory"); }

struct BnC { float mean, inv, ga, be; };
__device__ __forceinline__ BnC bn_c(const BnSet& s, int c) { return BnC{s.stat[2 * c], s.stat[2 * c + 1], s.gamma[c], s.beta[c]}; }
__device__ __forceinline__ float bn_act(float z, const BnC& k) { return fmaxf(fmaf(k.ga, (z - k.mean) * k.inv, k.be), 0.f); }
struct BnB { float mean, inv, ga, be, s1n, s2n; };
__device__ __forceinline__ BnB bn_b(const BnSet& s, int c, double count) {
  return BnB{s.stat[2 * c], s.stat[2 * c + 1], s.gamma[c], s.beta[c], (float)(s.bsums[2 * c] / count), (float)(s.bsums[2 * c + 1] / count)};
}
__device__ __forceinline__ float bn_dz(float da, float z, const BnB& k) {
  const float xh = (z - k.mean) * k.inv;
  const float dy = fmaf(k.ga, xh, k.be) > 0.f ? da : 0.f;
  return k.ga * k.inv * (dy - k.s1n - xh * k.s2n);
}

__device__ __forceinline__ void col_gemm(const float* xs, int x_off, int K, const float* W, int ldw, float (&acc)[kRC]) {
  const float* x = xs + x_off * kRC;
#pragma unroll 8
  for (int k = 0; k < K; ++k) {
    const float w = W[(int64_t)k * ldw];
    const float4 a = ld4(x + k * kRC), b = ld4(x + k * kRC + 4);
    acc[0] = fmaf(a.x, w, acc[0]); acc[1] = fmaf(a.y, w, acc[1]); acc[2] = fmaf(a.z, w, acc[2]); acc[3] = fmaf(a.w, w, acc[3]);
    acc[4] = fmaf(b.x, w, acc[4]); acc[5] = fmaf(b.y, w, acc[5]); acc[6] = fmaf(b.z, w, acc[6]); acc[7] = fmaf(b.w, w, acc[7]);
  }
}
__device__ __forceinline__ void acc_set(float (&acc)[kRC], float v) {
#pragma unroll
  for (int r = 0; r < kRC; ++r) acc[r] = v;
}

template <typename F>
__device__ __forceinline__ void stage_cols(float* __restrict__ xs, int x_off, const float* __restrict__ src, int ld, int C, int64_t row0, int nr, F f) {
  for (int c = threadIdx.x; c < C; c += kT2) {
    float v[kRC];
#pragma unroll
    for (int r = 0; r < kRC; ++r) v[r] = r < nr ? src[(row0 + r) * ld + c] : 0.f;
    float o[kRC];
    f(c, v, o);
#pragma unroll
    for (int r = 0; r < kRC; ++r) if (r >= nr) o[r] = 0.f;
    st4(xs + (x_off + c) * kRC, make_float4(o[0], o[1], o[2], o[3]));
    st4(xs + (x_off + c) * kRC + 4, make_float4(o[4], o[5], o[6], o[7]));
  }
}
__device__ __forceinline__ void stage_act(float* xs, int x_off, const float* Z, int ld, int C, int64_t row0, int nr, const BnSet& s) {
  stage_cols(xs, x_off, Z, ld, C, row0, nr, [&](int c, const float (&v)[kRC], float (&o)[kRC]) {
    const BnC k = bn_c(s, c);
#pragma unroll
    for (int r = 0; r < kRC; ++r) o[r] = bn_act(v[r], k);
  });
}
__device__ __forceinline__ void stage_dz(float* xs, int x_off, float* dA, const float* Z, int ld, int C, int64_t row0, int nr, const BnSet& s, double count) {
  for (int c = threadIdx.x; c < C; c += kT2) {
    const BnB k = bn_b(s, c, count);
    float o[kRC];
#pragma unroll
    for (int r = 0; r < kRC; ++r) {
      o[r] = 0.f;
      if (r < nr) {
        const int64_t i = (row0 + r) * ld + c;
        o[r] = bn_dz(dA[i], Z[i], k);
        dA[i] = o[r];
      }
    }
    st4(xs + (x_off + c) * kRC, make_float4(o[0], o[1], o[2], o[3]));
    st4(xs + (x_off + c) * kRC + 4, make_float4(o[4], o[5], o[6], o[7]));
  }
}

__device__ __forceinline__ void epi_fwd(const float (&acc)[kRC], float* __restrict__ Z, int ld, int col, int64_t row0, int nr, double& s, double& q) {
#pragma unroll
  for (int r = 0; r < kRC; ++r)
    if (r < nr) { Z[(row0 + r) * ld + col] = acc[r]; s += (double)acc[r]; q += (double)acc[r] * (double)acc[r]; }
}
__device__ __forceinline__ void epi_bwd(const float (&acc)[kRC], float* __restrict__ dA, const float* __restrict__ Zp, int ld, int col, int64_t row0, int nr,
                                        const BnC& k, double& s1, double& s2) {
#pragma unroll
  for (int r = 0; r < kRC; ++r)
    if (r < nr) {
      const int64_t i = (row0 + r) * ld + col;
      dA[i] = acc[r];
      const float xh = (Zp[i] - k.mean) * k.inv;
      const float dy = fmaf(k.ga, xh, k.be) > 0.f ? acc[r] : 0.f;
      s1 += (double)dy; s2 += (double)dy * (double)xh;
    }
}
__device__ __forceinline__ double* grp_fwd(const Head2& h, int set) { return h.gsums[set] + (size_t)(blockIdx.x % kHead2Groups) * 2 * h.bn[set].C; }
__device__ __forceinline__ double* grp_bwd(const Head2& h, int set) { return h.gbsums[set] + (size_t)(blockIdx.x % kHead2Groups) * 2 * h.bn[set].C; }
__device__ __forceinline__ void add_sums(double* dst, int col, double a, double b) {
  if (a != 0.0 || b != 0.0) { atomicAdd(dst + 2 * col, a); atomicAdd(dst + 2 * col + 1, b); }
}

struct Leader {
  int n_sync; int sync[2]; int bwd; int scalars;
  int fin_rows_n;
  int eval_stats;
};

__device__ __forceinline__ void leader_p2p(const HeadDyn& d, int slot, double* const* buf, const int* n, int nbuf) {
  const int tid = threadIdx.x;
  int total = 0;
  for (int b = 0; b < nbuf; ++b) total += n[b];
  const uint32_t ep = d.p2p_epoch;
  for (int i = tid; i < total; i += kT2) {
    int b = 0, o = i;
    while (o >= n[b]) { o -= n[b]; ++b; }
    const unsigned long long bits = (unsigned long long)__double_as_longlong(buf[b][o]);
    const uint4 v = make_uint4((uint32_t)bits, ep, (uint32_t)(bits >> 32), ep);
    for (int p = 0; p < d.world; ++p) {
      uint4* dst = d.peer_ll[p] + (size_t)(slot * d.world + d.rank) * kP2PMaxDoubles + i;
      asm volatile("st.relaxed.sys.global.v4.u32 [%0], {%1, %2, %3, %4};" ::"l"(dst), "r"(v.x), "r"(v.y), "r"(v.z), "r"(v.w) : "memory");
    }
  }
  const uint4* mine = d.peer_ll[d.rank] + (size_t)slot * d.world * kP2PMaxDoubles;
  for (int i = tid; i < total; i += kT2) {
    double s = 0.0;
    for (int p = 0; p < d.world; ++p) {
      const uint4* src = mine + (size_t)p * kP2PMaxDoubles + i;
      uint4 v;
      uint32_t spins = 0;
      for (;;) {
        asm volatile("ld.relaxed.sys.global.v4.u32 {%0, %1, %2, %3}, [%4];" : "=r"(v.x), "=r"(v.y), "=r"(v.z), "=r"(v.w) : "l"(src) : "memory");
        if (v.y == ep && v.w == ep) break;
        if (++spins > (1u << 22)) { *d.p2p_err = 1u + (uint32_t)slot; break; }
        __nanosleep(32);
      }
      s += __longlong_as_double((long long)(((unsigned long long)v.z << 32) | (unsigned long long)v.x));
    }
    int b = 0, o = i;
    while (o >= n[b]) { o -= n[b]; ++b; }
    buf[b][o] = s;
  }
  __syncthreads();
}

__device__ __forceinline__ double take_copies(double* g, int C, int i) {
  double v[kHead2Groups];
#pragma unroll
  for (int q = 0; q < kHead2Groups; ++q) v[q] = __ldcg(g + (size_t)q * 2 * C + i);
  double t = 0.0;
#pragma unroll
  for (int q = 0; q < kHead2Groups; ++q) { t += v[q]; g[(size_t)q * 2 * C + i] = 0.0; }
  return t;
}
__device__ __forceinline__ void bn_finalize_col(const BnSet& s, int c, double sum, double sq, double count, float mm, float mv) {
  const double mean = sum / count;
  double var = sq / count - mean * mean;
  if (var < 0.0) var = 0.0;
  s.stat[2 * c] = (float)mean;
  s.stat[2 * c + 1] = (float)(1.0 / sqrt(var + (double)kBnEps));
  s.mmean[c] = mm - (mm - (float)mean) * kBnDecay;
  s.mvar[c] = mv - (mv - (float)var) * kBnDecay;
}
__device__ __noinline__ void leader_work(const Head2& h, const HeadDyn& d, const Leader& L, int barrier_index) {
  const int tid = threadIdx.x;
  if (!d.training) {
    if (L.eval_stats)
      for (int k = 0; k < BN_COUNT; ++k) {
        const BnSet& s = h.bn[k];
        for (int c = tid; c < s.C; c += kT2) { s.stat[2 * c] = s.mmean[c]; s.stat[2 * c + 1] = 1.0f / sqrtf(s.mvar[c] + kBnEps); }
      }
    return;
  }
  const float gs = 1.0f / (float)d.world;
  if (d.world == 1) {
    for (int k = 0; k < L.n_sync; ++k) {
      const BnSet& s = h.bn[L.sync[k]];
      double* g = L.bwd ? h.gbsums[L.sync[k]] : h.gsums[L.sync[k]];
      const double count = L.fin_rows_n ? d.cntN : d.cntB;
      for (int c = tid; c < s.C; c += kT2) {
        float mm = 0.f, mv = 0.f;
        if (!L.bwd) { mm = __ldcg(s.mmean + c); mv = __ldcg(s.mvar + c); }
        const double a = take_copies(g, s.C, 2 * c), b = take_copies(g, s.C, 2 * c + 1);
        if (!L.bwd) bn_finalize_col(s, c, a, b, count, mm, mv);
        else {
          s.bsums[2 * c] = a; s.bsums[2 * c + 1] = b;
          s.dbeta[c] += (float)a * gs;
          s.dgamma[c] += (float)b * gs;
        }
      }
    }
    return;
  }
  for (int k = 0; k < L.n_sync; ++k) {
    const BnSet& s = h.bn[L.sync[k]];
    double* g = L.bwd ? h.gbsums[L.sync[k]] : h.gsums[L.sync[k]];
    double* dst = L.bwd ? s.bsums : s.sums;
    for (int i = tid; i < 2 * s.C; i += kT2) dst[i] = take_copies(g, s.C, i);
  }
  __syncthreads();
  if (L.n_sync > 0 || L.scalars) {
    double* buf[3]; int n[3]; int nb = 0;
    for (int k = 0; k < L.n_sync; ++k) { const BnSet& s = h.bn[L.sync[k]]; buf[nb] = L.bwd ? s.bsums : s.sums; n[nb++] = 2 * s.C; }
    if (L.scalars) { buf[nb] = h.dp_scalars; n[nb++] = 8; }
    leader_p2p(d, d.p2p_slot0 + barrier_index, buf, n, nb);
  }
  for (int k = 0; k < L.n_sync; ++k) {
    const BnSet& s = h.bn[L.sync[k]];
    if (!L.bwd) {
      const double count = L.fin_rows_n ? d.cntN : d.cntB;
      for (int c = tid; c < s.C; c += kT2) {
        bn_finalize_col(s, c, s.sums[2 * c], s.sums[2 * c + 1], count, s.mmean[c], s.mvar[c]);
        s.sums[2 * c] = 0.0;
        s.sums[2 * c + 1] = 0.0;
      }
    } else {
      for (int c = tid; c < s.C; c += kT2) {
        s.dbeta[c] += (float)s.bsums[2 * c] * gs;
        s.dgamma[c] += (float)s.bsums[2 * c + 1] * gs;
      }
    }
  }
}

struct Prefetch { const float* s0; int n0; const float* s1; int n1; };
__device__ __forceinline__ Prefetch no_prefetch() { return Prefetch{nullptr, 0, nullptr, 0}; }
__device__ __forceinline__ void copy_weights(float* __restrict__ wbuf, const Prefetch& pf, int t, int nt) {
#pragma unroll 1
  for (int part = 0; part < 2; ++part) {
    const float* __restrict__ src = part ? pf.s1 : pf.s0;
    const int n = part ? pf.n1 : pf.n0;
    float* dst = wbuf + (part ? pf.n0 : 0);
    for (int i0 = t; i0 < n; i0 += 16 * nt) {
      float v[16];
#pragma unroll
      for (int u = 0; u < 16; ++u) v[u] = i0 + u * nt < n ? __ldg(src + i0 + u * nt) : 0.f;
#pragma unroll
      for (int u = 0; u < 16; ++u) if (i0 + u * nt < n) dst[i0 + u * nt] = v[u];
    }
  }
}

__device__ __forceinline__ void grid_barrier(const Head2& h, const HeadDyn& d, unsigned& epoch, const Leader& L, int& n_barrier,
                                             float* wbuf, const Prefetch& pf) {
  unsigned* bar = d.bar;
  __syncthreads();
  if (d.trace_cta != nullptr && threadIdx.x == 0 && n_barrier < 16 && blockIdx.x < 256) {
    unsigned long long t; asm volatile("mov.u64 %0, %%globaltimer;" : "=l"(t)); d.trace_cta[n_barrier * 256 + blockIdx.x] = t;
  }
  if (blockIdx.x == 0) {
    if (threadIdx.x == 0) {
      unsigned spins = 0;
      while (ld_relaxed_u32(bar) < gridDim.x - 1) {
        if (++spins > (1u << 26)) { bar[2] = 1u + (unsigned)n_barrier; break; }
      }
      fence_acq_rel_gpu();
    } else if (gridDim.x == 1) {
      copy_weights(wbuf, pf, threadIdx.x - 1, kT2 - 1);
    }
    __syncthreads();
    leader_work(h, d, L, n_barrier);
    __syncthreads();
    if (threadIdx.x == 0) {
      if (d.trace != nullptr && n_barrier < 29) { unsigned long long t; asm volatile("mov.u64 %0, %%globaltimer;" : "=l"(t)); d.trace[n_barrier] = t; }
      bar[0] = 0u;
      __threadfence();
      st_release_u32(bar + 32, epoch + 1u);
    }
  } else {
    if (threadIdx.x == 0) {
      __threadfence();
      atomicAdd(bar, 1u);
      unsigned spins = 0;
      while ((int)(ld_relaxed_u32(bar + 32) - (epoch + 1u)) < 0) {
        if (++spins > (1u << 24)) { bar[2] = 1000u + (unsigned)n_barrier; break; }
        __nanosleep(32);
      }
      fence_acq_rel_gpu();
    } else {
      copy_weights(wbuf, pf, threadIdx.x - 1, kT2 - 1);
    }
    __syncthreads();
  }
  epoch += 1u;
  ++n_barrier;
}
__device__ __forceinline__ Leader leader_of(int a, int b, int bwd, int rows_n, int scalars = 0) {
  Leader L;
  L.n_sync = (a >= 0) + (b >= 0); L.sync[0] = a; L.sync[1] = b; L.bwd = bwd; L.scalars = scalars; L.fin_rows_n = rows_n; L.eval_stats = 0;
  return L;
}

__device__ __forceinline__ void pool_weights_w(const float* __restrict__ Z2, const BnC& k, const int* __restrict__ mask, int64_t base,
                                               int T, int lane, float* aw) {
  float s[8];
  float m = -INFINITY;
#pragma unroll
  for (int jj = 0; jj < 8; ++jj) {
    const int t = jj * 32 + lane;
    float val = -INFINITY;
    if (t < T) {
      const float sv = bn_act(Z2[base + t], k);
      val = (mask[base + t] == 1) ? sv : kMaskNeg;
    }
    s[jj] = val;
    m = fmaxf(m, val);
  }
  m = warp_max(m);
  float sum = 0.f;
#pragma unroll
  for (int jj = 0; jj < 8; ++jj) {
    const int t = jj * 32 + lane;
    const float e = (t < T) ? expf(s[jj] - m) : 0.f;
    s[jj] = e;
    sum += e;
  }
  sum = warp_sum(sum);
#pragma unroll
  for (int jj = 0; jj < 8; ++jj) {
    const int t = jj * 32 + lane;
    if (t < T) aw[t] = s[jj] / sum;
  }
  __syncwarp();
}

__device__ __forceinline__ double block_sum_d(double v, double* sh) {
  const int lane = threadIdx.x & 31, w = threadIdx.x >> 5;
  v = warp_sum_d(v);
  __syncthreads();
  if (lane == 0) sh[w] = v;
  __syncthreads();
  double r = 0.0;
#pragma unroll
  for (int k = 0; k < kT2 / 32; ++k) r += sh[k];
  return r;
}

__device__ __forceinline__ float sigm(float x) { return 1.0f / (1.0f + expf(-x)); }
__device__ __forceinline__ float xent(float x, float y) { return fmaxf(x, 0.f) - x * y + log1pf(expf(-fabsf(x))); }
__device__ __forceinline__ void loss_rows_item(const Head2& h, const HeadDyn& d, int item) {
  const int lane = threadIdx.x & 31, B = d.B;
  const float inv_b = 1.0f / (float)d.Bg;
  const int u = item * 32 + lane;
  double a0 = 0.0, a1 = 0.0;
  if (d.sm_group == 0) {
    const int b = u >> 1, head = u & 1;
    if (b < B) {
      const float x = h.logits[3 * b + head];
      const float y = head ? d.y_play[b] : d.y_sat[b];
      const double a = (double)xent(x, y);
      if (head) a1 = a; else a0 = a;
      h.d_logits[3 * b + head] = (head ? d.fuzhu_w : 1.0f) * (sigm(x) - y) * inv_b;
    }
  } else {
    const int sm = d.sm_group;
    const float scale = (float)sm * inv_b;
    if (u < 2 * (B / sm)) {
      const int head = u & 1, r0 = (u >> 1) * sm;
      const float* y = head ? d.y_play : d.y_sat;
      float mx = -INFINITY;
      for (int i = 0; i < sm; ++i) mx = fmaxf(mx, h.logits[3 * (r0 + i) + head]);
      float se = 0.f;
      int n_pos = 0;
      for (int i = 0; i < sm; ++i) { se += expf(h.logits[3 * (r0 + i) + head] - mx); n_pos += y[r0 + i] == 1.0f; }
      const float lse = mx + logf(se), wgt = head ? d.fuzhu_w : 1.0f;
      double acc = 0.0;
      for (int i = 0; i < sm; ++i) {
        const float x = h.logits[3 * (r0 + i) + head];
        const bool pos = y[r0 + i] == 1.0f;
        if (pos) acc += (double)(lse - x);
        h.d_logits[3 * (r0 + i) + head] = wgt * scale * ((float)n_pos * expf(x - lse) - (pos ? 1.0f : 0.f));
      }
      if (head) a1 = acc * (double)sm; else a0 = acc * (double)sm;
    }
  }
  if (item == 0) {
    const int G = B / PAMREC_GROUP;
    for (int b = G * 5 + lane; b < B; b += 32) h.d_logits[3 * b + 2] = 0.f;
  }
  a0 = warp_sum_d(a0); a1 = warp_sum_d(a1);
  if (lane == 0) {
    if (a0 != 0.0) atomicAdd(h.loss_acc, a0 / (double)d.Bg);
    if (a1 != 0.0) atomicAdd(h.loss_acc + 1, (double)d.fuzhu_w * a1 / (double)d.Bg);
  }
}
__device__ __forceinline__ void loss_ndcg_item(const Head2& h, const HeadDyn& d, int item) {
  const int lane = threadIdx.x & 31, sub = lane & 7, base = lane & ~7;
  const int G = d.B / PAMREC_GROUP;
  const int g = item * 4 + (lane >> 3);
  const bool on = g < G && sub < 5;
  const double nval = *h.dp_scalars;
  const float alpha = 10.0f;
  const int row = on ? g * 5 + sub : 0;
  const float s = on ? sigm(h.logits[3 * row + 2]) : 0.f;
  float y = on ? d.plays[row] : 0.f;
  float sj[5], yj[5];
#pragma unroll
  for (int j = 0; j < 5; ++j) { sj[j] = __shfl_sync(0xffffffffu, s, base + j); yj[j] = __shfl_sync(0xffffffffu, y, base + j); }
  const bool valid = (yj[0] + yj[1] + yj[2] + yj[3] + yj[4]) > 0.f;
  if (!valid) {
    y = 1e-10f;
#pragma unroll
    for (int j = 0; j < 5; ++j) yj[j] = 1e-10f;
  }
  const float gain = exp2f(y) - 1.0f;
  float rank = 1.0f, pq[5];
  int pos = 0;
#pragma unroll
  for (int j = 0; j < 5; ++j) {
    pq[j] = 0.f;
    if (j != sub) {
      const float p = sigm(alpha * (sj[j] - s));
      rank += p;
      pq[j] = p * (1.0f - p);
      pos += (yj[j] > y) || (yj[j] == y && j < sub);
    }
  }
  const float l1p = log1pf(rank);
  float dcg = on ? gain / l1p : 0.f, idcg = on ? gain / log1pf((float)(pos + 1)) : 0.f;
#pragma unroll
  for (int o = 4; o > 0; o >>= 1) { dcg += __shfl_xor_sync(0xffffffffu, dcg, o); idcg += __shfl_xor_sync(0xffffffffu, idcg, o); }
  const float inv = idcg > 0.f ? 1.0f / idcg : 0.f;
  const float w = valid ? 1.0f : 0.f;
  const float coef = (nval > 0.0) ? d.order_w * w / (float)nval : 0.f;
  const float dLr = gain * inv / (l1p * l1p * (1.0f + rank));
  float acc = 0.f;
#pragma unroll
  for (int j = 0; j < 5; ++j) {
    const float dj = __shfl_sync(0xffffffffu, dLr, base + j);
    acc += alpha * pq[j] * (dj - dLr);
  }
  if (on) h.d_logits[3 * row + 2] = coef * acc * s * (1.0f - s);
  double a2 = (on && sub == 0) ? (double)(w * -(dcg * inv)) : 0.0;
  a2 = warp_sum_d(a2);
  if (lane == 0 && a2 != 0.0 && nval > 0.0) atomicAdd(h.loss_acc + 2, (double)d.order_w * a2 / nval);
}

struct Rows { int b0, b1; };
__device__ __forceinline__ Rows my_rows(int B) {
  const int workers = max((int)gridDim.x - 1, 1);
  const int me = gridDim.x > 1 ? (int)blockIdx.x - 1 : 0;
  const int per = (B + workers - 1) / workers;
  Rows r;
  r.b0 = me < 0 ? B : min(B, me * per);
  r.b1 = me < 0 ? B : min(B, r.b0 + per);
  return r;
}

}

constexpr int kWT_t1 = 0;
constexpr int kWT_t0 = kWT_t1 + 3 * 6400;
constexpr int kWT_e1 = kWT_t0 + 3 * 8400;
constexpr int kWT_g1 = kWT_e1 + 5 * 6400;
constexpr int kWT_x0 = kWT_g1 + 2 * 320;
constexpr int kWT_total = kWT_x0 + 628 * 40;
static_assert(kWT_total == kHead2WtFloats, "head2.h: workspace size of the transposed weights");
__device__ __forceinline__ void head2_transpose_weights(const Head2& h) {
  float* wT = h.wT;
  const int64_t gtid = (int64_t)blockIdx.x * kT2 + threadIdx.x, gsz = (int64_t)gridDim.x * kT2;
  for (int64_t i = gtid; i < kWT_total; i += gsz) {
    float v;
    if (i < kWT_t0) { const int j = (int)i, g = j / 6400, r = j % 6400, n = r / 100, k = r % 100; v = h.t_w1[g * 6400 + k * 64 + n]; }
    else if (i < kWT_e1) { const int j = (int)i - kWT_t0, g = j / 8400, r = j % 8400, n = r / 84, k = r % 84; v = h.t_w0[g * 8400 + k * 100 + n]; }
    else if (i < kWT_g1) { const int j = (int)i - kWT_e1, g = j / 6400, r = j % 6400, n = r / 100, k = r % 100; v = h.e_w1[g * 6400 + k * 64 + n]; }
    else if (i < kWT_x0) { const int j = (int)i - kWT_g1, g = j / 320, r = j % 320, n = r / 64, k = r % 64; v = h.g_w1[g * 320 + k * 5 + n]; }
    else {
      const int j = (int)i - kWT_x0, row = j / 40, k = j % 40;
      if (row < 500) { const int g = row / 100, n = row % 100; v = h.e_w0[g * 4000 + k * 100 + n]; }
      else { const int rr = row - 500, g = rr / 64, n = rr % 64; v = h.g_w0[g * 2560 + k * 64 + n]; }
    }
    wT[i] = v;
  }
}

__global__ void __launch_bounds__(kT2, 1) k_head2_fwd(const __grid_constant__ Head2 h, const __grid_constant__ HeadDyn d) {
  extern __shared__ __align__(16) float dsm[];
  float* wbuf = dsm;
  float* xs = dsm + kWBuf;
  __shared__ __align__(16) float w0s[kD * 20 + 64];
  __shared__ double shd[64];
  __shared__ unsigned s_epoch;
  const int tid = threadIdx.x, lane = tid & 31, warp = tid >> 5;
  if (tid == 0 && blockIdx.x == 0 && d.trace != nullptr) { unsigned long long t; asm volatile("mov.u64 %0, %%globaltimer;" : "=l"(t)); d.trace[31] = t; }
  if (tid == 0) s_epoch = ld_relaxed_u32(d.bar + 32);
  for (int i = tid; i < kD * 20; i += kT2) w0s[i] = h.s_w0[i];
  if (tid < 20) { w0s[800 + tid] = h.s_b0[tid]; w0s[820 + tid] = h.s_w1[tid]; }
  if (tid == 0) w0s[840] = h.s_b1[0];
  __syncthreads();
  unsigned epoch = s_epoch;
  int n_barrier = 0;
  const bool train = d.training != 0;
  const int T = d.T;
  const Rows R = my_rows(d.B);
  const int64_t tok0 = (int64_t)R.b0 * T, tok1 = (int64_t)R.b1 * T;
  auto sync_point = [&](const Leader& L, const Prefetch& pf) {
    if (train) grid_barrier(h, d, epoch, L, n_barrier, wbuf, pf);
    else { __syncthreads(); copy_weights(wbuf, pf, tid, kT2); __syncthreads(); }
  };
  if (!train) { Leader L = leader_of(-1, -1, 0, 0); L.eval_stats = 1; grid_barrier(h, d, epoch, L, n_barrier, wbuf, no_prefetch()); }

  if (train && blockIdx.x == 0) {
    const int G = d.B / PAMREC_GROUP;
    double cnt = 0.0;
    for (int g = tid; g < G; g += kT2) {
      float sg = 0.f;
#pragma unroll
      for (int i = 0; i < PAMREC_GROUP; ++i) sg += d.plays[g * PAMREC_GROUP + i];
      cnt += (sg > 0.f) ? 1.0 : 0.0;
    }
    cnt = block_sum_d(cnt, shd);
    if (tid == 0) h.dp_scalars[0] = cnt;
  }
  {
    constexpr int kChunk = 5 * kSlots;
    const int slot = tid / 20, j = tid % 20;
    double s = 0.0, q = 0.0;
    float wc[kD];
#pragma unroll
    for (int k = 0; k < kD; ++k) wc[k] = w0s[k * 20 + (slot < kSlots ? j : 0)];
    const float b = w0s[800 + j];
    float4 pre[3];
    auto load_chunk = [&](int64_t c0) {
      const int nq = (int)min((int64_t)kChunk, tok1 - c0) * 10;
#pragma unroll
      for (int u = 0; u < 3; ++u) { const int i = tid + u * kT2; pre[u] = i < nq ? ld4(h.H + c0 * kD + 4 * i) : f4_zero(); }
    };
    if (tok0 < tok1) load_chunk(tok0);
    for (int64_t c0 = tok0; c0 < tok1; c0 += kChunk) {
      const int nt = (int)min((int64_t)kChunk, tok1 - c0);
      __syncthreads();
#pragma unroll
      for (int u = 0; u < 3; ++u) { const int i = tid + u * kT2; if (i < kChunk * 10) st4(xs + 4 * i, pre[u]); }
      __syncthreads();
      if (c0 + kChunk < tok1) load_chunk(c0 + kChunk);
      if (slot < kSlots) {
#pragma unroll
        for (int u = 0; u < 5; ++u) {
          const int tl = slot + u * kSlots;
          if (tl < nt) {
            const float* hr = xs + tl * kD;
            float z = b;
#pragma unroll
            for (int i = 0; i < 10; ++i) {
              const float4 x = ld4(hr + 4 * i);
              z = fmaf(x.x, wc[4 * i], z); z = fmaf(x.y, wc[4 * i + 1], z); z = fmaf(x.z, wc[4 * i + 2], z); z = fmaf(x.w, wc[4 * i + 3], z);
            }
            h.z1[(c0 + tl) * 20 + j] = z;
            s += (double)z; q += (double)z * (double)z;
          }
        }
      }
    }
    __syncthreads();
    if (train) {
      double* red = reinterpret_cast<double*>(xs);
      if (slot < kSlots) { red[slot * 20 + j] = s; red[500 + slot * 20 + j] = q; }
      __syncthreads();
      if (tid < 40) {
        const int which = tid / 20, c = tid % 20;
        double t = 0.0;
        for (int k = 0; k < kSlots; ++k) t += red[which * 500 + k * 20 + c];
        if (t != 0.0) atomicAdd(grp_fwd(h, BN_S0) + 2 * c + which, t);
      }
    }
    sync_point(leader_of(BN_S0, -1, 0, 1, 1), Prefetch{h.e_w0, 5 * 4000, h.g_w0, 2 * 2560});
  }
  __syncthreads();
  {
    const BnSet& s0 = h.bn[BN_S0];
    double s = 0.0, q = 0.0;
    for (int64_t tok = tok0 + tid; tok < tok1; tok += kT2) {
      const float* zr = h.z1 + tok * 20;
      float z = w0s[840];
#pragma unroll
      for (int i = 0; i < 5; ++i) {
        const float4 x = ld4(zr + 4 * i);
        z = fmaf(bn_act(x.x, bn_c(s0, 4 * i)), w0s[820 + 4 * i], z);
        z = fmaf(bn_act(x.y, bn_c(s0, 4 * i + 1)), w0s[820 + 4 * i + 1], z);
        z = fmaf(bn_act(x.z, bn_c(s0, 4 * i + 2)), w0s[820 + 4 * i + 2], z);
        z = fmaf(bn_act(x.w, bn_c(s0, 4 * i + 3)), w0s[820 + 4 * i + 3], z);
      }
      h.z2[tok] = z;
      s += (double)z; q += (double)z * (double)z;
    }
    if (train) {
      s = block_sum_d(s, shd); q = block_sum_d(q, shd);
      if (tid == 0 && (s != 0.0 || q != 0.0)) { atomicAdd(grp_fwd(h, BN_S1), s); atomicAdd(grp_fwd(h, BN_S1) + 1, q); }
    }
    sync_point(leader_of(BN_S1, -1, 0, 1), no_prefetch());
  }
  __syncthreads();
  {
    const BnC k1 = bn_c(h.bn[BN_S1], 0);
    float* aws = xs;
    for (int b = R.b0 + warp; b < R.b1; b += kT2 / 32) {
      const int64_t base = (int64_t)b * T;
      float* aw = aws + warp * PAMREC_MAX_T;
      pool_weights_w(h.z2, k1, d.mask, base, T, lane, aw);
      const int tg = lane / 10, c = lane % 10;
      float4 acc = f4_zero();
      if (lane < 30)
        for (int t = tg; t < T; t += 3) f4_fma(acc, aw[t], ld4(h.H + (base + t) * kD + 4 * c));
      const float4 a1 = f4_shfl_down(acc, 10), a2 = f4_shfl_down(acc, 20);
      if (lane < 10) {
        acc.x += a1.x + a2.x; acc.y += a1.y + a2.y; acc.z += a1.z + a2.z; acc.w += a1.w + a2.w;
        st4(h.new_long + (int64_t)b * kD + 4 * c, acc);
      }
      if (train) for (int t = lane; t < T; t += 32) h.aw[base + t] = aw[t];
      __syncwarp();
    }
    __syncthreads();
    double s[2] = {0.0, 0.0}, q[2] = {0.0, 0.0};
    for (int row0 = R.b0; row0 < R.b1; row0 += kRC) {
      const int nr = min(kRC, R.b1 - row0);
      __syncthreads();
      stage_cols(xs, 0, h.new_long, kD, kD, row0, nr, [](int, const float (&v)[kRC], float (&o)[kRC]) {
#pragma unroll
        for (int r = 0; r < kRC; ++r) o[r] = v[r];
      });
      __syncthreads();
#pragma unroll
      for (int pass = 0; pass < 2; ++pass) {
        const int col = tid + pass * kT2;
        if (col >= 628) continue;
        float acc[kRC];
        if (col < 500) {
          const int g = col / 100, n = col % 100;
          acc_set(acc, h.e_b0[g * 100 + n]);
          col_gemm(xs, 0, kD, wbuf + g * 4000 + n, 100, acc);
          epi_fwd(acc, h.ze0, 500, col, row0, nr, s[pass], q[pass]);
        } else {
          const int cg = col - 500, g = cg / 64, n = cg % 64;
          acc_set(acc, h.g_b0[g * 64 + n]);
          col_gemm(xs, 0, kD, wbuf + 20000 + g * 2560 + n, 64, acc);
          epi_fwd(acc, h.zg0, 128, cg, row0, nr, s[pass], q[pass]);
        }
      }
    }
    if (train) {
#pragma unroll
      for (int pass = 0; pass < 2; ++pass) {
        const int col = tid + pass * kT2;
        if (col < 500) add_sums(grp_fwd(h, BN_E0), col, s[pass], q[pass]);
        else if (col < 628) add_sums(grp_fwd(h, BN_G0), col - 500, s[pass], q[pass]);
      }
    }
    sync_point(leader_of(BN_E0, BN_G0, 0, 0), Prefetch{h.e_w1, 5 * 6400, h.g_w1, 2 * 320});
  }
  {
    double s = 0.0, q = 0.0;
    for (int row0 = R.b0; row0 < R.b1; row0 += kRC) {
      const int nr = min(kRC, R.b1 - row0);
      __syncthreads();
      stage_act(xs, 0, h.ze0, 500, 500, row0, nr, h.bn[BN_E0]);
      stage_act(xs, 500, h.zg0, 128, 128, row0, nr, h.bn[BN_G0]);
      __syncthreads();
      const int col = tid;
      float acc[kRC];
      if (col < 320) {
        const int g = col / 64, n = col % 64;
        acc_set(acc, h.e_b1[g * 64 + n]);
        col_gemm(xs, g * 100, 100, wbuf + g * 6400 + n, 64, acc);
        epi_fwd(acc, h.ze1, 320, col, row0, nr, s, q);
      } else if (col < 330) {
        const int cg = col - 320, g = cg / 5, n = cg % 5;
        acc_set(acc, h.g_b1[g * 5 + n]);
        col_gemm(xs, 500 + g * 64, 64, wbuf + 32000 + g * 320 + n, 5, acc);
        epi_fwd(acc, h.zg1, 10, cg, row0, nr, s, q);
      }
    }
    if (train) {
      if (tid < 320) add_sums(grp_fwd(h, BN_E1), tid, s, q);
      else if (tid < 330) add_sums(grp_fwd(h, BN_G1), tid - 320, s, q);
    }
    sync_point(leader_of(BN_E1, BN_G1, 0, 0), Prefetch{h.t_w0, 3 * 8400, nullptr, 0});
  }
  {
    double s = 0.0, q = 0.0;
    float* es = xs + 168 * kRC;
    for (int row0 = R.b0; row0 < R.b1; row0 += kRC) {
      const int nr = min(kRC, R.b1 - row0);
      __syncthreads();
      stage_act(es, 0, h.ze1, 320, 320, row0, nr, h.bn[BN_E1]);
      stage_act(es, 320, h.zg1, 10, 10, row0, nr, h.bn[BN_G1]);
      __syncthreads();
      if (tid < 168) {
        const int c = tid;
        float o[kRC];
        if (c < 64 || (c >= 84 && c < 148)) {
          const int cc = c < 64 ? c : c - 84, gb = c < 64 ? 0 : 5;
#pragma unroll
          for (int r = 0; r < kRC; ++r) {
            float m = 0.f;
#pragma unroll
            for (int j = 0; j < 5; ++j) m = fmaf(es[(320 + gb + j) * kRC + r], es[(j * 64 + cc) * kRC + r], m);
            o[r] = m;
          }
        } else {
          const int cc = c < 84 ? c - 64 : c - 148;
#pragma unroll
          for (int r = 0; r < kRC; ++r) o[r] = r < nr ? h.tgt[(int64_t)(row0 + r) * kE + cc] : 0.f;
        }
#pragma unroll
        for (int r = 0; r < kRC; ++r) {
          if (r >= nr) o[r] = 0.f; else h.u[(int64_t)(row0 + r) * 168 + c] = o[r];
        }
        st4(xs + c * kRC, make_float4(o[0], o[1], o[2], o[3]));
        st4(xs + c * kRC + 4, make_float4(o[4], o[5], o[6], o[7]));
      }
      __syncthreads();
      if (tid < 300) {
        const int g = tid / 100, n = tid % 100;
        float acc[kRC];
        acc_set(acc, h.t_b0[g * 100 + n]);
        col_gemm(xs, g == 1 ? 84 : 0, 84, wbuf + g * 8400 + n, 100, acc);
        epi_fwd(acc, h.zt0, 300, tid, row0, nr, s, q);
      }
    }
    if (train && tid < 300) add_sums(grp_fwd(h, BN_T0), tid, s, q);
    sync_point(leader_of(BN_T0, -1, 0, 0), Prefetch{h.t_w1, 3 * 6400, nullptr, 0});
  }
  {
    double s = 0.0, q = 0.0;
    for (int row0 = R.b0; row0 < R.b1; row0 += kRC) {
      const int nr = min(kRC, R.b1 - row0);
      __syncthreads();
      stage_act(xs, 0, h.zt0, 300, 300, row0, nr, h.bn[BN_T0]);
      __syncthreads();
      if (tid < 192) {
        const int g = tid / 64, n = tid % 64;
        float acc[kRC];
        acc_set(acc, h.t_b1[g * 64 + n]);
        col_gemm(xs, g * 100, 100, wbuf + g * 6400 + n, 64, acc);
        epi_fwd(acc, h.zt1, 192, tid, row0, nr, s, q);
      }
    }
    if (train && tid < 192) add_sums(grp_fwd(h, BN_T1), tid, s, q);
    sync_point(leader_of(BN_T1, -1, 0, 0), no_prefetch());
  }
  {
    for (int row0 = R.b0; row0 < R.b1; row0 += kRC) {
      const int nr = min(kRC, R.b1 - row0);
      __syncthreads();
      stage_act(xs, 0, h.zt1, 192, 192, row0, nr, h.bn[BN_T1]);
      __syncthreads();
      if (tid < 3 * kRC) {
        const int g = tid / kRC, r = tid % kRC;
        if (r < nr) {
          float z = h.t_bo[g];
          for (int k = 0; k < 64; ++k) z = fmaf(xs[(g * 64 + k) * kRC + r], h.t_wo[g * 64 + k], z);
          h.logits[(int64_t)(row0 + r) * 3 + g] = z;
          if (g == 0 && d.pred != nullptr) d.pred[row0 + r] = sigm(z);
        }
      }
    }
  }
  if (tid == 0 && blockIdx.x == 0 && d.trace != nullptr) { unsigned long long t; asm volatile("mov.u64 %0, %%globaltimer;" : "=l"(t)); d.trace[30] = t; d.trace[29] = (unsigned long long)n_barrier; }
  if (train) head2_transpose_weights(h);
}

__global__ void __launch_bounds__(kT2, 1) k_head2_bwd(const __grid_constant__ Head2 h, const __grid_constant__ HeadDyn d) {
  extern __shared__ __align__(16) float dsm[];
  float* wbuf = dsm;
  float* xs = dsm + kWBuf;
  float* aux = xs + kXS * kRC;
  __shared__ double shd[64];
  __shared__ unsigned s_epoch;
  const int tid = threadIdx.x, lane = tid & 31, warp = tid >> 5;
  if (tid == 0 && blockIdx.x == 0 && d.trace != nullptr) { unsigned long long t; asm volatile("mov.u64 %0, %%globaltimer;" : "=l"(t)); d.trace[31] = t; }
  if (tid == 0) s_epoch = ld_relaxed_u32(d.bar + 32);
  __syncthreads();
  unsigned epoch = s_epoch;
  int n_barrier = 0;
  const int T = d.T;
  const Rows R = my_rows(d.B);
  const int64_t tok0 = (int64_t)R.b0 * T, tok1 = (int64_t)R.b1 * T;
  const float* wT = h.wT;

  {
    const int G = d.B / PAMREC_GROUP;
    const int n_ndcg = (G + 3) / 4;
    const int n_units = d.sm_group > 0 ? 2 * (d.B / d.sm_group) : 2 * d.B;
    const int n_rows = max((n_units + 31) / 32, 1);
    const int workers = max((int)gridDim.x - 1, 1), me = gridDim.x > 1 ? (int)blockIdx.x - 1 : 0;
    if (d.B > 0 && me >= 0)
      for (int i = me + workers * warp; i < n_ndcg + n_rows; i += workers * (kT2 / 32)) {
        if (i < n_ndcg) loss_ndcg_item(h, d, i); else loss_rows_item(h, d, i - n_ndcg);
      }
    grid_barrier(h, d, epoch, leader_of(-1, -1, 1, 0), n_barrier, wbuf, Prefetch{wT + kWT_t1, 3 * 6400, nullptr, 0});
  }
  {
    double s1 = 0.0, s2 = 0.0;
    if (tid < 192) {
      const int g = tid / 64, n = tid % 64;
      const float w = h.t_wo[g * 64 + n];
      const BnC k = bn_c(h.bn[BN_T1], tid);
      for (int b = R.b0; b < R.b1; ++b) {
        const int64_t i = (int64_t)b * 192 + tid;
        const float da = h.d_logits[(int64_t)b * 3 + g] * w;
        h.d_t1[i] = da;
        const float xh = (h.zt1[i] - k.mean) * k.inv;
        const float dy = fmaf(k.ga, xh, k.be) > 0.f ? da : 0.f;
        s1 += (double)dy; s2 += (double)dy * (double)xh;
      }
      add_sums(grp_bwd(h, BN_T1), tid, s1, s2);
    }
    grid_barrier(h, d, epoch, leader_of(BN_T1, -1, 1, 0), n_barrier, wbuf, no_prefetch());
  }
  {
    double s1 = 0.0, s2 = 0.0;
    const BnC k = tid < 300 ? bn_c(h.bn[BN_T0], tid) : BnC{0.f, 0.f, 0.f, 0.f};
    for (int row0 = R.b0; row0 < R.b1; row0 += kRC) {
      const int nr = min(kRC, R.b1 - row0);
      __syncthreads();
      stage_dz(xs, 0, h.d_t1, h.zt1, 192, 192, row0, nr, h.bn[BN_T1], d.cntB);
      __syncthreads();
      if (tid < 300) {
        const int g = tid / 100, kk = tid % 100;
        float acc[kRC];
        acc_set(acc, 0.f);
        col_gemm(xs, g * 64, 64, wbuf + g * 6400 + kk, 100, acc);
        epi_bwd(acc, h.d_t0, h.zt0, 300, tid, row0, nr, k, s1, s2);
      }
    }
    if (tid < 300) add_sums(grp_bwd(h, BN_T0), tid, s1, s2);
    grid_barrier(h, d, epoch, leader_of(BN_T0, -1, 1, 0), n_barrier, wbuf, Prefetch{wT + kWT_t0, 3 * 8400, nullptr, 0});
  }
  {
    double s1 = 0.0, s2 = 0.0;
    const BnC k = tid < 320 ? bn_c(h.bn[BN_E1], tid) : BnC{0.f, 0.f, 0.f, 0.f};
    const BnC kg = (tid >= 320 && tid < 400) ? bn_c(h.bn[BN_G1], (tid - 320) >> 3) : BnC{0.f, 0.f, 0.f, 0.f};
    float* du = aux;
    float* gt = aux + 168 * kRC;
    for (int row0 = R.b0; row0 < R.b1; row0 += kRC) {
      const int nr = min(kRC, R.b1 - row0);
      __syncthreads();
      stage_dz(xs, 0, h.d_t0, h.zt0, 300, 300, row0, nr, h.bn[BN_T0], d.cntB);
      stage_act(gt, 0, h.zg1, 10, 10, row0, nr, h.bn[BN_G1]);
      stage_act(xs, 300, h.ze1, 320, 320, row0, nr, h.bn[BN_E1]);
      __syncthreads();
      if (tid < 168) {
        float acc[kRC];
        acc_set(acc, 0.f);
        if (tid < 84) {
          col_gemm(xs, 0, 100, wbuf + tid, 84, acc);
          col_gemm(xs, 200, 100, wbuf + 2 * 8400 + tid, 84, acc);
        } else {
          col_gemm(xs, 100, 100, wbuf + 8400 + (tid - 84), 84, acc);
        }
        st4(du + tid * kRC, make_float4(acc[0], acc[1], acc[2], acc[3]));
        st4(du + tid * kRC + 4, make_float4(acc[4], acc[5], acc[6], acc[7]));
      }
      __syncthreads();
      if (tid >= 480 && tid < 500) {
        const int c = tid - 480;
        for (int r = 0; r < nr; ++r) h.d_tgt[(int64_t)(row0 + r) * kE + c] = du[(64 + c) * kRC + r] + du[(148 + c) * kRC + r];
      }
      if (tid < 320) {
        const int j = tid / 64, c = tid % 64;
#pragma unroll
        for (int r = 0; r < kRC; ++r)
          if (r < nr) {
            const int64_t i = (int64_t)(row0 + r) * 320 + tid;
            const float da = gt[j * kRC + r] * du[c * kRC + r] + gt[(5 + j) * kRC + r] * du[(84 + c) * kRC + r];
            h.d_e1[i] = da;
            const float xh = (h.ze1[i] - k.mean) * k.inv;
            const float dy = fmaf(k.ga, xh, k.be) > 0.f ? da : 0.f;
            s1 += (double)dy; s2 += (double)dy * (double)xh;
          }
      } else if (tid < 400) {
        const int jj = (tid - 320) >> 3, r = (tid - 320) & 7, j = jj % 5, off = jj < 5 ? 0 : 84;
        if (r < nr) {
          float da = 0.f;
          for (int c = 0; c < 64; ++c) da = fmaf(xs[(300 + j * 64 + c) * kRC + r], du[(off + c) * kRC + r], da);
          const int64_t i = (int64_t)(row0 + r) * 10 + jj;
          h.d_g1[i] = da;
          const float xh = (h.zg1[i] - kg.mean) * kg.inv;
          const float dy = fmaf(kg.ga, xh, kg.be) > 0.f ? da : 0.f;
          s1 += (double)dy; s2 += (double)dy * (double)xh;
        }
      }
    }
    if (tid < 320) add_sums(grp_bwd(h, BN_E1), tid, s1, s2);
    else if (tid < 400) add_sums(grp_bwd(h, BN_G1), (tid - 320) >> 3, s1, s2);
    grid_barrier(h, d, epoch, leader_of(BN_E1, BN_G1, 1, 0), n_barrier, wbuf, Prefetch{wT + kWT_e1, 5 * 6400 + 2 * 320, nullptr, 0});
  }
  {
    double s1[2] = {0.0, 0.0}, s2[2] = {0.0, 0.0};
    BnC kc[2];
#pragma unroll
    for (int pass = 0; pass < 2; ++pass) {
      const int col = tid + pass * kT2;
      kc[pass] = col < 500 ? bn_c(h.bn[BN_E0], col) : (col < 628 ? bn_c(h.bn[BN_G0], col - 500) : BnC{0.f, 0.f, 0.f, 0.f});
    }
    for (int row0 = R.b0; row0 < R.b1; row0 += kRC) {
      const int nr = min(kRC, R.b1 - row0);
      __syncthreads();
      stage_dz(xs, 0, h.d_e1, h.ze1, 320, 320, row0, nr, h.bn[BN_E1], d.cntB);
      stage_dz(xs, 320, h.d_g1, h.zg1, 10, 10, row0, nr, h.bn[BN_G1], d.cntB);
      __syncthreads();
#pragma unroll
      for (int pass = 0; pass < 2; ++pass) {
        const int col = tid + pass * kT2;
        if (col >= 628) continue;
        float acc[kRC];
        acc_set(acc, 0.f);
        if (col < 500) {
          const int g = col / 100, kk = col % 100;
          col_gemm(xs, g * 64, 64, wbuf + g * 6400 + kk, 100, acc);
          epi_bwd(acc, h.d_e0, h.ze0, 500, col, row0, nr, kc[pass], s1[pass], s2[pass]);
        } else {
          const int cg = col - 500, g = cg / 64, kk = cg % 64;
          col_gemm(xs, 320 + g * 5, 5, wbuf + 32000 + g * 320 + kk, 64, acc);
          epi_bwd(acc, h.d_g0, h.zg0, 128, cg, row0, nr, kc[pass], s1[pass], s2[pass]);
        }
      }
    }
#pragma unroll
    for (int pass = 0; pass < 2; ++pass) {
      const int col = tid + pass * kT2;
      if (col < 500) add_sums(grp_bwd(h, BN_E0), col, s1[pass], s2[pass]);
      else if (col < 628) add_sums(grp_bwd(h, BN_G0), col - 500, s1[pass], s2[pass]);
    }
    grid_barrier(h, d, epoch, leader_of(BN_E0, BN_G0, 1, 0), n_barrier, wbuf, Prefetch{wT + kWT_x0, 628 * 40, nullptr, 0});
  }
  {
    const BnC k1 = bn_c(h.bn[BN_S1], 0);
    double b1 = 0.0, b2 = 0.0;
    float* part = aux;
    float* dnl = xs;
    for (int row0 = R.b0; row0 < R.b1; row0 += kRC) {
      const int nr = min(kRC, R.b1 - row0);
      __syncthreads();
      stage_dz(xs, 0, h.d_e0, h.ze0, 500, 500, row0, nr, h.bn[BN_E0], d.cntB);
      stage_dz(xs, 500, h.d_g0, h.zg0, 128, 128, row0, nr, h.bn[BN_G0], d.cntB);
      __syncthreads();
      if (tid < 480) {
        const int grp = tid / 40, c = tid % 40;
        const int k0 = grp * 53, kn = min(53, 628 - k0);
        float acc[kRC];
        acc_set(acc, 0.f);
        col_gemm(xs, k0, kn, wbuf + k0 * 40 + c, 40, acc);
        float* p = part + (grp * 40 + c) * kRC;
        st4(p, make_float4(acc[0], acc[1], acc[2], acc[3]));
        st4(p + 4, make_float4(acc[4], acc[5], acc[6], acc[7]));
      }
      __syncthreads();
      if (tid < 40 * kRC) {
        const int r = tid / 40, c = tid % 40;
        float v = 0.f;
#pragma unroll
        for (int g = 0; g < 12; ++g) v += part[(g * 40 + c) * kRC + r];
        dnl[r * 40 + c] = v;
        if (r < nr) h.d_new_long[(int64_t)(row0 + r) * kD + c] = v;
      }
      __syncthreads();
      if (warp < nr) {
        const int b = row0 + warp;
        const int64_t base = (int64_t)b * T;
        float4 dn[10];
#pragma unroll
        for (int i = 0; i < 10; ++i) dn[i] = ld4(dnl + warp * 40 + 4 * i);
        float da[8], a[8];
        float dot = 0.f;
#pragma unroll
        for (int jj = 0; jj < 8; ++jj) {
          const int t = jj * 32 + lane;
          float v = 0.f, av = 0.f;
          if (t < T) {
            const float* hr = h.H + (base + t) * kD;
#pragma unroll
            for (int i = 0; i < 10; ++i) v += f4_dot(dn[i], ld4(hr + 4 * i));
            av = h.aw[base + t];
            dot = fmaf(av, v, dot);
          }
          da[jj] = v; a[jj] = av;
        }
        dot = warp_sum(dot);
#pragma unroll
        for (int jj = 0; jj < 8; ++jj) {
          const int t = jj * 32 + lane;
          if (t < T) {
            const float dv = (d.mask[base + t] == 1) ? a[jj] * (da[jj] - dot) : 0.f;
            h.d_z2[base + t] = dv;
            const float xh = (h.z2[base + t] - k1.mean) * k1.inv;
            const float dy = fmaf(k1.ga, xh, k1.be) > 0.f ? dv : 0.f;
            b1 += (double)dy; b2 += (double)dy * (double)xh;
          }
        }
      }
    }
    b1 = block_sum_d(b1, shd); b2 = block_sum_d(b2, shd);
    if (tid == 0 && (b1 != 0.0 || b2 != 0.0)) { atomicAdd(grp_bwd(h, BN_S1), b1); atomicAdd(grp_bwd(h, BN_S1) + 1, b2); }
    grid_barrier(h, d, epoch, leader_of(BN_S1, -1, 1, 1), n_barrier, wbuf, no_prefetch());
  }
  float* w0s = aux;
  float* w0t = aux + 800;
  float* w1s = aux + 1600;
  float* c0 = aux + 1620;
  __syncthreads();
  for (int i = tid; i < 800; i += kT2) { const float v = h.s_w0[i]; w0s[i] = v; w0t[(i % 20) * 40 + i / 20] = v; }
  if (tid < 20) w1s[tid] = h.s_w1[tid];
  {
    const BnB k1 = bn_b(h.bn[BN_S1], 0, d.cntN);
    const int slot = tid / 20, j = tid % 20;
    double s1 = 0.0, s2 = 0.0, gw = 0.0, gb = 0.0;
    __syncthreads();
    if (slot < kSlots) {
      const BnC k0 = bn_c(h.bn[BN_S0], j);
      const float w1j = w1s[j];
      for (int64_t tok = tok0 + slot; tok < tok1; tok += kSlots) {
        const float dz2 = bn_dz(h.d_z2[tok], h.z2[tok], k1);
        const float xh = (h.z1[tok * 20 + j] - k0.mean) * k0.inv;
        const float y = fmaf(k0.ga, xh, k0.be);
        gw += (double)(fmaxf(y, 0.f) * dz2);
        if (j == 0) gb += (double)dz2;
        const float dy = y > 0.f ? dz2 * w1j : 0.f;
        s1 += (double)dy; s2 += (double)dy * (double)xh;
      }
    }
    double* red = reinterpret_cast<double*>(xs);
    __syncthreads();
    if (slot < kSlots) { red[slot * 20 + j] = s1; red[500 + slot * 20 + j] = s2; red[1000 + slot * 20 + j] = gw; red[1500 + slot * 20 + j] = gb; }
    __syncthreads();
    if (tid < 80) {
      const int which = tid / 20, c = tid % 20;
      double t = 0.0;
      for (int k = 0; k < kSlots; ++k) t += red[which * 500 + k * 20 + c];
      if (t != 0.0) {
        if (which < 2) atomicAdd(grp_bwd(h, BN_S0) + 2 * c + which, t);
        else if (which == 2) atomicAdd(h.ds_w1 + c, (float)t);
        else if (c == 0) atomicAdd(h.ds_b1, (float)t);
      }
    }
    grid_barrier(h, d, epoch, leader_of(BN_S0, -1, 1, 1), n_barrier, wbuf, no_prefetch());
  }
  {
    constexpr int kTB = 2 * kSlots;
    const BnB k1 = bn_b(h.bn[BN_S1], 0, d.cntN);
    const int slot = tid / 20, j = tid % 20;
    const int sl_h = tid / 10, kq = tid % 10;
    if (tid < 20) {
      const BnB k = bn_b(h.bn[BN_S0], tid, d.cntN);
      c0[6 * tid] = k.mean; c0[6 * tid + 1] = k.inv; c0[6 * tid + 2] = k.ga; c0[6 * tid + 3] = k.be; c0[6 * tid + 4] = k.s1n; c0[6 * tid + 5] = k.s2n;
    }
    float* Hs = xs;
    float* dzs = xs + kTB * kD;
    float gw[4] = {0.f, 0.f, 0.f, 0.f};
    double gb = 0.0;
    const int wk = tid / 5, wjq = tid % 5;
    __syncthreads();
    const bool colthr = slot < kSlots;
    const BnB k0 = colthr ? BnB{c0[6 * j], c0[6 * j + 1], c0[6 * j + 2], c0[6 * j + 3], c0[6 * j + 4], c0[6 * j + 5]} : BnB{0.f, 0.f, 0.f, 0.f, 0.f, 0.f};
    const float w1j = colthr ? w1s[j] : 0.f;
    float4 pH = f4_zero(), pDn = f4_zero();
    float pA = 0.f, pdA[2] = {0.f, 0.f}, pz2[2] = {0.f, 0.f}, pz1[2] = {0.f, 0.f};
    auto prefetch = [&](int64_t tb) {
      const int nt = (int)min((int64_t)kTB, tok1 - tb);
      if (tid < kTB * 10) {
        const bool ok = sl_h < nt;
        const int64_t tok = tb + sl_h;
        pH = ok ? ld4(h.H + tok * kD + 4 * kq) : f4_zero();
        pA = ok ? h.aw[tok] : 0.f;
        pDn = ok ? ld4(h.d_new_long + (tok / T) * kD + 4 * kq) : f4_zero();
      }
      if (colthr) {
#pragma unroll
        for (int u = 0; u < 2; ++u) {
          const int sl = slot + u * kSlots;
          const int64_t tok = tb + sl;
          pdA[u] = sl < nt ? h.d_z2[tok] : 0.f; pz2[u] = sl < nt ? h.z2[tok] : 0.f; pz1[u] = sl < nt ? h.z1[tok * 20 + j] : 0.f;
        }
      }
    };
    if (tok0 < tok1) prefetch(tok0);
    for (int64_t tb = tok0; tb < tok1; tb += kTB) {
      const int nt = (int)min((int64_t)kTB, tok1 - tb);
      __syncthreads();
      float4 dn = pDn;
      const float a = pA;
      if (tid < kTB * 10) st4(Hs + 4 * tid, pH);
      if (colthr) {
#pragma unroll
        for (int u = 0; u < 2; ++u) {
          const int sl = slot + u * kSlots;
          float dz1 = 0.f;
          if (sl < nt) {
            const float dz2 = bn_dz(pdA[u], pz2[u], k1);
            dz1 = bn_dz(dz2 * w1j, pz1[u], k0);
            gb += (double)dz1;
          }
          dzs[sl * 20 + j] = dz1;
        }
      }
      __syncthreads();
      if (tb + kTB < tok1) prefetch(tb + kTB);
      if (tid < kTB * 10 && sl_h < nt) {
        float4 o = make_float4(a * dn.x, a * dn.y, a * dn.z, a * dn.w);
#pragma unroll
        for (int jj = 0; jj < 20; ++jj) f4_fma(o, dzs[sl_h * 20 + jj], ld4(w0t + jj * 40 + 4 * kq));
        st4(h.g_a + (tb + sl_h) * kD + 4 * kq, o);
      }
      if (tid < 200) {
        float4 acc = make_float4(gw[0], gw[1], gw[2], gw[3]);
#pragma unroll 5
        for (int sl = 0; sl < nt; ++sl) f4_fma(acc, Hs[sl * 40 + wk], ld4(dzs + sl * 20 + 4 * wjq));
        gw[0] = acc.x; gw[1] = acc.y; gw[2] = acc.z; gw[3] = acc.w;
      }
    }
    if (tid < 200) {
#pragma unroll
      for (int i = 0; i < 4; ++i) if (gw[i] != 0.f) atomicAdd(h.ds_w0 + wk * 20 + 4 * wjq + i, gw[i]);
    }
    double* red = reinterpret_cast<double*>(aux + 2048);
    __syncthreads();
    if (colthr) red[slot * 20 + j] = gb;
    __syncthreads();
    if (tid < 20) {
      double t = 0.0;
      for (int k = 0; k < kSlots; ++k) t += red[k * 20 + tid];
      if (t != 0.0) atomicAdd(h.ds_b0 + tid, (float)t);
    }
  }
  if (tid == 0 && blockIdx.x == 0 && d.trace != nullptr) { unsigned long long t; asm volatile("mov.u64 %0, %%globaltimer;" : "=l"(t)); d.trace[30] = t; d.trace[29] = (unsigned long long)n_barrier; }
}

namespace {
constexpr int kDwThreads = 128;
constexpr int kDwRows = 64;
struct DwProb {
  const float* X; int ldx; int x_off0, x_stride;
  int x_mod;
  int bn;
  const float* dZ; int lddz; int z_stride;
  int K, N, groups;
  float* dW; int w_stride; float* db; int b_stride;
  int kblocks, first_task;
};
struct DwPlan { DwProb p[7]; int n_prob; int splits; int total; };
}

__global__ void __launch_bounds__(kDwThreads) k_head2_dw(const __grid_constant__ Head2 h, const __grid_constant__ DwPlan plan, int B) {
  __shared__ __align__(16) float xsm[kDwRows * 8];
  const int tid = threadIdx.x;
  int task = blockIdx.x / plan.splits;
  const int split = blockIdx.x % plan.splits;
  int pi = 0;
  while (pi + 1 < plan.n_prob && task >= plan.p[pi + 1].first_task) ++pi;
  const DwProb& P = plan.p[pi];
  task -= P.first_task;
  const int g = task / P.kblocks, kb = task % P.kblocks;
  const int k0 = kb * 8, kn = min(8, P.K - k0);
  const int xo = (P.x_mod ? (g * P.x_stride) % P.x_mod : P.x_off0 + g * P.x_stride) + k0;
  const int zo = g * P.z_stride;
  const int rows_per = (B + plan.splits - 1) / plan.splits;
  const int r_begin = split * rows_per, r_end = min(B, r_begin + rows_per);
  float acc[8] = {0.f, 0.f, 0.f, 0.f, 0.f, 0.f, 0.f, 0.f};
  float sb = 0.f;
  const int n = tid;
  for (int r0 = r_begin; r0 < r_end; r0 += kDwRows) {
    const int nr = min(kDwRows, r_end - r0);
    __syncthreads();
    for (int i = tid; i < kDwRows * 8; i += kDwThreads) {
      const int r = i >> 3, kk = i & 7;
      float v = 0.f;
      if (r < nr && kk < kn) {
        v = P.X[(int64_t)(r0 + r) * P.ldx + xo + kk];
        if (P.bn >= 0) v = bn_act(v, bn_c(h.bn[P.bn], xo + kk));
      }
      xsm[i] = v;
    }
    __syncthreads();
    if (n < P.N) {
      const float* dz = P.dZ + (int64_t)r0 * P.lddz + zo + n;
#pragma unroll 4
      for (int r = 0; r < nr; ++r) {
        const float z = dz[(int64_t)r * P.lddz];
        const float4 a = ld4(xsm + r * 8), b = ld4(xsm + r * 8 + 4);
        acc[0] = fmaf(a.x, z, acc[0]); acc[1] = fmaf(a.y, z, acc[1]); acc[2] = fmaf(a.z, z, acc[2]); acc[3] = fmaf(a.w, z, acc[3]);
        acc[4] = fmaf(b.x, z, acc[4]); acc[5] = fmaf(b.y, z, acc[5]); acc[6] = fmaf(b.z, z, acc[6]); acc[7] = fmaf(b.w, z, acc[7]);
        sb += z;
      }
    }
  }
  if (n < P.N) {
    float* dW = P.dW + (int64_t)g * P.w_stride + (int64_t)k0 * P.N + n;
#pragma unroll
    for (int i = 0; i < 8; ++i) if (i < kn) atomicAdd(dW + (int64_t)i * P.N, acc[i]);
    if (kb == 0) atomicAdd(P.db + (int64_t)g * P.b_stride + n, sb);
  }
}

constexpr size_t kFwdSmem = (size_t)(kWBuf + kXS * kRC) * sizeof(float);
constexpr size_t kBwdSmem = (size_t)(kWBuf + kXS * kRC + 4096) * sizeof(float);
int head2_grid() {
  int dev = 0, sms = 0, coop = 0, occ_f = 0, occ_b = 0;
  if (cudaGetDevice(&dev) != cudaSuccess) return -1;
  if (cudaFuncSetAttribute(k_head2_fwd, cudaFuncAttributeMaxDynamicSharedMemorySize, (int)kFwdSmem) != cudaSuccess) return -1;
  if (cudaFuncSetAttribute(k_head2_bwd, cudaFuncAttributeMaxDynamicSharedMemorySize, (int)kBwdSmem) != cudaSuccess) return -1;
  if (cudaDeviceGetAttribute(&sms, cudaDevAttrMultiProcessorCount, dev) != cudaSuccess) return -1;
  cudaDeviceGetAttribute(&coop, cudaDevAttrCooperativeLaunch, dev);
  if (!coop) return -1;
  if (cudaOccupancyMaxActiveBlocksPerMultiprocessor(&occ_f, k_head2_fwd, kT2, kFwdSmem) != cudaSuccess || occ_f < 1) return -1;
  if (cudaOccupancyMaxActiveBlocksPerMultiprocessor(&occ_b, k_head2_bwd, kT2, kBwdSmem) != cudaSuccess || occ_b < 1) return -1;
  return sms;
}

int launch_head2_fwd(const Head2& h, const HeadDyn& d, int grid, const char* name, cudaStream_t st) {
  PAMREC_PROF(name, 1, st);
  if (d.B == 0 && d.world == 1) return 0;
  void* args[2] = {(void*)&h, (void*)&d};
  return cudaLaunchCooperativeKernel((const void*)k_head2_fwd, dim3(grid), dim3(kT2), args, kFwdSmem, st) == cudaSuccess ? 0 : -1;
}
int launch_head2_bwd(const Head2& h, const HeadDyn& d, int grid, cudaStream_t st) {
  PAMREC_PROF("head_bwd", 1, st);
  if (d.B == 0 && d.world == 1) return 0;
  void* args[2] = {(void*)&h, (void*)&d};
  return cudaLaunchCooperativeKernel((const void*)k_head2_bwd, dim3(grid), dim3(kT2), args, kBwdSmem, st) == cudaSuccess ? 0 : -1;
}
void launch_head2_dw(const Head2& h, int B, cudaStream_t st) {
  PAMREC_PROF("head_dw", 1, st);
  if (B == 0) return;
  DwPlan pl;
  memset(&pl, 0, sizeof pl);
  auto add = [&](const float* X, int ldx, int x_stride, int x_mod, int bn, const float* dZ, int lddz, int z_stride, int K, int N, int groups,
                 float* dW, int w_stride, float* db, int b_stride) {
    DwProb& p = pl.p[pl.n_prob++];
    p.X = X; p.ldx = ldx; p.x_off0 = 0; p.x_stride = x_stride; p.x_mod = x_mod; p.bn = bn; p.dZ = dZ; p.lddz = lddz; p.z_stride = z_stride;
    p.K = K; p.N = N; p.groups = groups; p.dW = dW; p.w_stride = w_stride; p.db = db; p.b_stride = b_stride;
    p.kblocks = (K + 7) / 8; p.first_task = pl.total;
    pl.total += groups * p.kblocks;
  };
  add(h.zt1, 192, 64, 0, BN_T1, h.d_logits, 3, 1, 64, 1, 3, h.dt_wo, 64, h.dt_bo, 1);
  add(h.zt0, 300, 100, 0, BN_T0, h.d_t1, 192, 64, 100, 64, 3, h.dt_w1, 6400, h.dt_b1, 64);
  add(h.u, 168, 84, 168, -1, h.d_t0, 300, 100, 84, 100, 3, h.dt_w0, 8400, h.dt_b0, 100);
  add(h.ze0, 500, 100, 0, BN_E0, h.d_e1, 320, 64, 100, 64, 5, h.de_w1, 6400, h.de_b1, 64);
  add(h.zg0, 128, 64, 0, BN_G0, h.d_g1, 10, 5, 64, 5, 2, h.dg_w1, 320, h.dg_b1, 5);
  add(h.new_long, kD, 0, 0, -1, h.d_e0, 500, 100, kD, 100, 5, h.de_w0, 4000, h.de_b0, 100);
  add(h.new_long, kD, 0, 0, -1, h.d_g0, 128, 64, kD, 64, 2, h.dg_w0, 2560, h.dg_b0, 64);
  pl.splits = (B + 255) / 256;
  if (pl.splits > 64) pl.splits = 64;
  k_head2_dw<<<pl.total * pl.splits, kDwThreads, 0, st>>>(h, pl, B);
}

}
```

Before: 1.380 million.

## Replace leader-serialized grid barrier with flat counter barrier and redundant per-block BN finalize

In single-GPU training the cooperative head kernels now sync through a flat 64-bit arrival counter instead of a leader block that waits, finalizes batch-norm statistics and then releases the rest. After the barrier every block sums the per-group BN partial copies itself and writes mean/invstd (or normalized bsums) into a new shared-memory table. Only block 0 writes the canonical globals and clears the previous stage's copies lazily. This takes the serial leader phase and the second round-trip off the critical path, at the cost of redundant reductions in every block and extra shared memory per block.

```diff
diff --git a/pamrec_b200/csrc/api.cu b/pamrec_b200/csrc/api.cu
--- a/pamrec_b200/csrc/api.cu
+++ b/pamrec_b200/csrc/api.cu
@@ -737,6 +737,7 @@
   H.wT = h->wf("head.wT");
   static_assert(kHead2Groups == 8, "layout.h: bn.gsums / bn.gbsums hold 8 copies");
   for (int i = 0; i < BN_COUNT; ++i) {
+    if (h->bn[i].C != kHead2BnCols[i]) return fail(h, "head2: batch-norm set %d has %d channels, the kernels expect %d", i, h->bn[i].C, kHead2BnCols[i]);
     H.bn[i] = h->bn[i];
     H.gsums[i] = h->wd("bn.gsums") + (size_t)kHead2Groups * L.bn_bsums_off[i];
     H.gbsums[i] = h->wd("bn.gbsums") + (size_t)kHead2Groups * L.bn_bsums_off[i];
diff --git a/pamrec_b200/csrc/head2.h b/pamrec_b200/csrc/head2.h
--- a/pamrec_b200/csrc/head2.h
+++ b/pamrec_b200/csrc/head2.h
@@ -7,6 +7,8 @@
 constexpr int kHead2Threads = 512;
 constexpr int kHead2Groups = 8;
 constexpr int kHead2WtFloats = 3 * 6400 + 3 * 8400 + 5 * 6400 + 2 * 320 + 628 * 40;
+constexpr int kHead2BnCols[BN_COUNT] = {20, 1, 500, 128, 320, 10, 300, 192};
+constexpr int kHead2BnTotal = 1471;
 
 struct Head2 {
   const float* H;
diff --git a/pamrec_b200/csrc/kernels_head2.cu b/pamrec_b200/csrc/kernels_head2.cu
--- a/pamrec_b200/csrc/kernels_head2.cu
+++ b/pamrec_b200/csrc/kernels_head2.cu
@@ -16,6 +16,11 @@
 __device__ __forceinline__ unsigned ld_relaxed_u32(const unsigned* p) {
   unsigned v;
   asm volatile("ld.relaxed.gpu.global.u32 %0, [%1];" : "=r"(v) : "l"(p) : "memory");
+  return v;
+}
+__device__ __forceinline__ unsigned long long ld_relaxed_u64(const unsigned long long* p) {
+  unsigned long long v;
+  asm volatile("ld.relaxed.gpu.global.u64 %0, [%1];" : "=l"(v) : "l"(p) : "memory");
   return v;
 }
 __device__ __forceinline__ void fence_acq_rel_gpu() { asm volatile("fence.acq_rel.gpu;" ::: "memory"); }
@@ -27,12 +32,23 @@
 }
 __device__ __forceinline__ void fence_acq_rel_sys() { asm volatile("fence.acq_rel.sys;" ::: "memory"); }
 
+__host__ __device__ constexpr int bn_off(int set) {
+  return (set > BN_S0) * 20 + (set > BN_S1) * 1 + (set > BN_E0) * 500 + (set > BN_G0) * 128 + (set > BN_E1) * 320 + (set > BN_G1) * 10 +
+         (set > BN_T0) * 300;
+}
+static_assert(bn_off(BN_S1) == kHead2BnCols[BN_S0] && bn_off(BN_E0) == bn_off(BN_S1) + kHead2BnCols[BN_S1] &&
+              bn_off(BN_G0) == bn_off(BN_E0) + kHead2BnCols[BN_E0] && bn_off(BN_E1) == bn_off(BN_G0) + kHead2BnCols[BN_G0] &&
+              bn_off(BN_G1) == bn_off(BN_E1) + kHead2BnCols[BN_E1] && bn_off(BN_T0) == bn_off(BN_G1) + kHead2BnCols[BN_G1] &&
+              bn_off(BN_T1) == bn_off(BN_T0) + kHead2BnCols[BN_T0] && kHead2BnTotal == bn_off(BN_T1) + kHead2BnCols[BN_T1],
+              "head2.h: kHead2BnCols");
+__device__ __forceinline__ float* bn_sh(float* bns, int set) { return bns + 2 * bn_off(set); }
 struct BnC { float mean, inv, ga, be; };
-__device__ __forceinline__ BnC bn_c(const BnSet& s, int c) { return BnC{s.stat[2 * c], s.stat[2 * c + 1], s.gamma[c], s.beta[c]}; }
+__device__ __forceinline__ BnC bn_c(const BnSet& s, const float* st, int c) { return BnC{st[2 * c], st[2 * c + 1], s.gamma[c], s.beta[c]}; }
+__device__ __forceinline__ BnC bn_c(const BnSet& s, int c) { return bn_c(s, s.stat, c); }
 __device__ __forceinline__ float bn_act(float z, const BnC& k) { return fmaxf(fmaf(k.ga, (z - k.mean) * k.inv, k.be), 0.f); }
 struct BnB { float mean, inv, ga, be, s1n, s2n; };
-__device__ __forceinline__ BnB bn_b(const BnSet& s, int c, double count) {
-  return BnB{s.stat[2 * c], s.stat[2 * c + 1], s.gamma[c], s.beta[c], (float)(s.bsums[2 * c] / count), (float)(s.bsums[2 * c + 1] / count)};
+__device__ __forceinline__ BnB bn_b(const BnSet& s, const float* sn, int c) {
+  return BnB{s.stat[2 * c], s.stat[2 * c + 1], s.gamma[c], s.beta[c], sn[2 * c], sn[2 * c + 1]};
 }
 __device__ __forceinline__ float bn_dz(float da, float z, const BnB& k) {
   const float xh = (z - k.mean) * k.inv;
@@ -69,16 +85,18 @@
     st4(xs + (x_off + c) * kRC + 4, make_float4(o[4], o[5], o[6], o[7]));
   }
 }
-__device__ __forceinline__ void stage_act(float* xs, int x_off, const float* Z, int ld, int C, int64_t row0, int nr, const BnSet& s) {
+__device__ __forceinline__ void stage_act(float* xs, int x_off, const float* Z, int ld, int C, int64_t row0, int nr, const BnSet& s,
+                                          const float* st) {
   stage_cols(xs, x_off, Z, ld, C, row0, nr, [&](int c, const float (&v)[kRC], float (&o)[kRC]) {
-    const BnC k = bn_c(s, c);
+    const BnC k = bn_c(s, st, c);
 #pragma unroll
     for (int r = 0; r < kRC; ++r) o[r] = bn_act(v[r], k);
   });
 }
-__device__ __forceinline__ void stage_dz(float* xs, int x_off, float* dA, const float* Z, int ld, int C, int64_t row0, int nr, const BnSet& s, double count) {
+__device__ __forceinline__ void stage_dz(float* xs, int x_off, float* dA, const float* Z, int ld, int C, int64_t row0, int nr, const BnSet& s,
+                                         const float* sn) {
   for (int c = threadIdx.x; c < C; c += kT2) {
-    const BnB k = bn_b(s, c, count);
+    const BnB k = bn_b(s, sn, c);
     float o[kRC];
 #pragma unroll
     for (int r = 0; r < kRC; ++r) {
@@ -119,9 +137,16 @@
 
 struct Leader {
   int n_sync; int sync[2]; int bwd; int scalars;
-  int fin_rows_n;
   int eval_stats;
 };
+struct Grid {
+  unsigned epoch;
+  unsigned long long base;
+  int n;
+  Leader prev;
+};
+__device__ __forceinline__ double bn_count(const HeadDyn& d, int set) { return (set == BN_S0 || set == BN_S1) ? d.cntN : d.cntB; }
+__device__ __forceinline__ double* copies_of(const Head2& h, int set, int bwd) { return bwd ? h.gbsums[set] : h.gsums[set]; }
 
 __device__ __forceinline__ void leader_p2p(const HeadDyn& d, int slot, double* const* buf, const int* n, int nbuf) {
   const int tid = threadIdx.x;
@@ -160,24 +185,30 @@
   __syncthreads();
 }
 
-__device__ __forceinline__ double take_copies(double* g, int C, int i) {
+__device__ __forceinline__ double sum_copies(const double* g, int C, int i) {
   double v[kHead2Groups];
 #pragma unroll
   for (int q = 0; q < kHead2Groups; ++q) v[q] = __ldcg(g + (size_t)q * 2 * C + i);
   double t = 0.0;
 #pragma unroll
-  for (int q = 0; q < kHead2Groups; ++q) { t += v[q]; g[(size_t)q * 2 * C + i] = 0.0; }
+  for (int q = 0; q < kHead2Groups; ++q) t += v[q];
   return t;
 }
-__device__ __forceinline__ void bn_finalize_col(const BnSet& s, int c, double sum, double sq, double count, float mm, float mv) {
-  const double mean = sum / count;
-  double var = sq / count - mean * mean;
+__device__ __forceinline__ void zero_copies(double* g, int C) {
+  for (int i = threadIdx.x; i < kHead2Groups * 2 * C; i += kT2) g[i] = 0.0;
+}
+__device__ __forceinline__ void bn_moments(double sum, double sq, double count, double& mean, double& var) {
+  mean = sum / count;
+  var = sq / count - mean * mean;
   if (var < 0.0) var = 0.0;
-  s.stat[2 * c] = (float)mean;
-  s.stat[2 * c + 1] = (float)(1.0 / sqrt(var + (double)kBnEps));
+}
+__device__ __forceinline__ float bn_invstd(double var) { return (float)(1.0 / sqrt(var + (double)kBnEps)); }
+__device__ __forceinline__ void bn_moving(const BnSet& s, int c, double mean, double var) {
+  const float mm = s.mmean[c], mv = s.mvar[c];
   s.mmean[c] = mm - (mm - (float)mean) * kBnDecay;
   s.mvar[c] = mv - (mv - (float)var) * kBnDecay;
 }
+
 __device__ __noinline__ void leader_work(const Head2& h, const HeadDyn& d, const Leader& L, int barrier_index) {
   const int tid = threadIdx.x;
   if (!d.training) {
@@ -189,30 +220,13 @@
     return;
   }
   const float gs = 1.0f / (float)d.world;
-  if (d.world == 1) {
-    for (int k = 0; k < L.n_sync; ++k) {
-      const BnSet& s = h.bn[L.sync[k]];
-      double* g = L.bwd ? h.gbsums[L.sync[k]] : h.gsums[L.sync[k]];
-      const double count = L.fin_rows_n ? d.cntN : d.cntB;
-      for (int c = tid; c < s.C; c += kT2) {
-        float mm = 0.f, mv = 0.f;
-        if (!L.bwd) { mm = __ldcg(s.mmean + c); mv = __ldcg(s.mvar + c); }
-        const double a = take_copies(g, s.C, 2 * c), b = take_copies(g, s.C, 2 * c + 1);
-        if (!L.bwd) bn_finalize_col(s, c, a, b, count, mm, mv);
-        else {
-          s.bsums[2 * c] = a; s.bsums[2 * c + 1] = b;
-          s.dbeta[c] += (float)a * gs;
-          s.dgamma[c] += (float)b * gs;
-        }
-      }
-    }
-    return;
-  }
   for (int k = 0; k < L.n_sync; ++k) {
     const BnSet& s = h.bn[L.sync[k]];
-    double* g = L.bwd ? h.gbsums[L.sync[k]] : h.gsums[L.sync[k]];
+    double* g = copies_of(h, L.sync[k], L.bwd);
     double* dst = L.bwd ? s.bsums : s.sums;
-    for (int i = tid; i < 2 * s.C; i += kT2) dst[i] = take_copies(g, s.C, i);
+    for (int i = tid; i < 2 * s.C; i += kT2) dst[i] = sum_copies(g, s.C, i);
+    __syncthreads();
+    zero_copies(g, s.C);
   }
   __syncthreads();
   if (L.n_sync > 0 || L.scalars) {
@@ -224,9 +238,13 @@
   for (int k = 0; k < L.n_sync; ++k) {
     const BnSet& s = h.bn[L.sync[k]];
     if (!L.bwd) {
-      const double count = L.fin_rows_n ? d.cntN : d.cntB;
+      const double count = bn_count(d, L.sync[k]);
       for (int c = tid; c < s.C; c += kT2) {
-        bn_finalize_col(s, c, s.sums[2 * c], s.sums[2 * c + 1], count, s.mmean[c], s.mvar[c]);
+        double mean, var;
+        bn_moments(s.sums[2 * c], s.sums[2 * c + 1], count, mean, var);
+        s.stat[2 * c] = (float)mean;
+        s.stat[2 * c + 1] = bn_invstd(var);
+        bn_moving(s, c, mean, var);
         s.sums[2 * c] = 0.0;
         s.sums[2 * c + 1] = 0.0;
       }
@@ -257,39 +275,79 @@
   }
 }
 
-__device__ __forceinline__ void grid_barrier(const Head2& h, const HeadDyn& d, unsigned& epoch, const Leader& L, int& n_barrier,
-                                             float* wbuf, const Prefetch& pf) {
+__device__ __forceinline__ unsigned long long globaltimer() { unsigned long long t; asm volatile("mov.u64 %0, %%globaltimer;" : "=l"(t)); return t; }
+__device__ __forceinline__ unsigned long long* flat_counter(const HeadDyn& d) { return reinterpret_cast<unsigned long long*>(d.bar + 48); }
+__device__ __forceinline__ bool flat_mode(const HeadDyn& d) { return d.training && d.world == 1; }
+__device__ __forceinline__ void trace_arrival(const HeadDyn& d, int n) {
+  if (d.trace_cta != nullptr && threadIdx.x == 0 && n < 15 && blockIdx.x < 256) d.trace_cta[n * 256 + blockIdx.x] = globaltimer();
+}
+
+__device__ __forceinline__ Grid grid_start(const HeadDyn& d, unsigned long long* sh) {
+  if (threadIdx.x == 0) {
+    if (d.trace_cta != nullptr && blockIdx.x < 256) d.trace_cta[15 * 256 + blockIdx.x] = globaltimer();
+    const unsigned long long v = ld_relaxed_u64(flat_counter(d));
+    sh[0] = v - v % gridDim.x;
+    sh[1] = ld_relaxed_u32(d.bar + 32);
+  }
+  __syncthreads();
+  Grid g;
+  g.base = sh[0]; g.epoch = (unsigned)sh[1]; g.n = 0;
+  g.prev.n_sync = 0; g.prev.bwd = 0; g.prev.scalars = 0; g.prev.eval_stats = 0;
+  __syncthreads();
+  return g;
+}
+
+__device__ __forceinline__ void flat_barrier(const HeadDyn& d, Grid& G, float* wbuf, const Prefetch& pf) {
+  __syncthreads();
+  trace_arrival(d, G.n);
+  if (threadIdx.x == 0) {
+    unsigned long long* ctr = flat_counter(d);
+    const unsigned long long target = G.base + (unsigned long long)(G.n + 1) * gridDim.x;
+    __threadfence();
+    atomicAdd(ctr, 1ull);
+    unsigned spins = 0;
+    while (ld_relaxed_u64(ctr) < target) {
+      if (++spins > (1u << 24)) { d.bar[2] = 2000u + (unsigned)G.n; break; }
+      __nanosleep(32);
+    }
+    fence_acq_rel_gpu();
+    if (blockIdx.x == 0 && d.trace != nullptr && G.n < 29) d.trace[G.n] = globaltimer();
+  } else {
+    copy_weights(wbuf, pf, threadIdx.x - 1, kT2 - 1);
+  }
+  __syncthreads();
+}
+
+__device__ __forceinline__ void leader_barrier(const Head2& h, const HeadDyn& d, Grid& G, const Leader& L, float* wbuf, const Prefetch& pf) {
   unsigned* bar = d.bar;
   __syncthreads();
-  if (d.trace_cta != nullptr && threadIdx.x == 0 && n_barrier < 16 && blockIdx.x < 256) {
-    unsigned long long t; asm volatile("mov.u64 %0, %%globaltimer;" : "=l"(t)); d.trace_cta[n_barrier * 256 + blockIdx.x] = t;
-  }
+  trace_arrival(d, G.n);
   if (blockIdx.x == 0) {
     if (threadIdx.x == 0) {
       unsigned spins = 0;
       while (ld_relaxed_u32(bar) < gridDim.x - 1) {
-        if (++spins > (1u << 26)) { bar[2] = 1u + (unsigned)n_barrier; break; }
+        if (++spins > (1u << 26)) { bar[2] = 1u + (unsigned)G.n; break; }
       }
       fence_acq_rel_gpu();
     } else if (gridDim.x == 1) {
       copy_weights(wbuf, pf, threadIdx.x - 1, kT2 - 1);
     }
     __syncthreads();
-    leader_work(h, d, L, n_barrier);
+    leader_work(h, d, L, G.n);
     __syncthreads();
     if (threadIdx.x == 0) {
-      if (d.trace != nullptr && n_barrier < 29) { unsigned long long t; asm volatile("mov.u64 %0, %%globaltimer;" : "=l"(t)); d.trace[n_barrier] = t; }
+      if (d.trace != nullptr && G.n < 29) d.trace[G.n] = globaltimer();
       bar[0] = 0u;
       __threadfence();
-      st_release_u32(bar + 32, epoch + 1u);
+      st_release_u32(bar + 32, G.epoch + 1u);
     }
   } else {
     if (threadIdx.x == 0) {
       __threadfence();
       atomicAdd(bar, 1u);
       unsigned spins = 0;
-      while ((int)(ld_relaxed_u32(bar + 32) - (epoch + 1u)) < 0) {
-        if (++spins > (1u << 24)) { bar[2] = 1000u + (unsigned)n_barrier; break; }
+      while ((int)(ld_relaxed_u32(bar + 32) - (G.epoch + 1u)) < 0) {
+        if (++spins > (1u << 24)) { bar[2] = 1000u + (unsigned)G.n; break; }
         __nanosleep(32);
       }
       fence_acq_rel_gpu();
@@ -298,12 +356,58 @@
     }
     __syncthreads();
   }
-  epoch += 1u;
-  ++n_barrier;
-}
-__device__ __forceinline__ Leader leader_of(int a, int b, int bwd, int rows_n, int scalars = 0) {
+  G.epoch += 1u;
+}
+
+__device__ __forceinline__ void grid_sync(const Head2& h, const HeadDyn& d, Grid& G, const Leader& L, float* bns, float* wbuf, const Prefetch& pf) {
+  const int tid = threadIdx.x;
+  if (flat_mode(d)) {
+    flat_barrier(d, G, wbuf, pf);
+    const bool canon = blockIdx.x == 0;
+    for (int k = 0; k < L.n_sync; ++k) {
+      const int set = L.sync[k];
+      const BnSet& s = h.bn[set];
+      const double* g = copies_of(h, set, L.bwd);
+      const double count = bn_count(d, set);
+      float* o = bn_sh(bns, set);
+      for (int c = tid; c < s.C; c += kT2) {
+        const double a = sum_copies(g, s.C, 2 * c), b = sum_copies(g, s.C, 2 * c + 1);
+        if (!L.bwd) {
+          double mean, var;
+          bn_moments(a, b, count, mean, var);
+          o[2 * c] = (float)mean;
+          o[2 * c + 1] = bn_invstd(var);
+          if (canon) { s.stat[2 * c] = o[2 * c]; s.stat[2 * c + 1] = o[2 * c + 1]; bn_moving(s, c, mean, var); }
+        } else {
+          o[2 * c] = (float)(a / count);
+          o[2 * c + 1] = (float)(b / count);
+          if (canon) { s.bsums[2 * c] = a; s.bsums[2 * c + 1] = b; s.dbeta[c] += (float)a; s.dgamma[c] += (float)b; }
+        }
+      }
+    }
+    if (canon)
+      for (int k = 0; k < G.prev.n_sync; ++k) zero_copies(copies_of(h, G.prev.sync[k], G.prev.bwd), h.bn[G.prev.sync[k]].C);
+    G.prev = L;
+  } else {
+    leader_barrier(h, d, G, L, wbuf, pf);
+    for (int k = 0; k < BN_COUNT; ++k) {
+      const bool all = L.eval_stats, mine = (L.n_sync > 0 && L.sync[0] == k) || (L.n_sync > 1 && L.sync[1] == k);
+      if (!all && !mine) continue;
+      const BnSet& s = h.bn[k];
+      float* o = bn_sh(bns, k);
+      const double count = bn_count(d, k);
+      for (int c = tid; c < s.C; c += kT2) {
+        if (!L.bwd) { o[2 * c] = __ldcg(s.stat + 2 * c); o[2 * c + 1] = __ldcg(s.stat + 2 * c + 1); }
+        else { o[2 * c] = (float)(__ldcg(s.bsums + 2 * c) / count); o[2 * c + 1] = (float)(__ldcg(s.bsums + 2 * c + 1) / count); }
+      }
+    }
+  }
+  __syncthreads();
+  ++G.n;
+}
+__device__ __forceinline__ Leader leader_of(int a, int b, int bwd, int scalars = 0) {
   Leader L;
-  L.n_sync = (a >= 0) + (b >= 0); L.sync[0] = a; L.sync[1] = b; L.bwd = bwd; L.scalars = scalars; L.fin_rows_n = rows_n; L.eval_stats = 0;
+  L.n_sync = (a >= 0) + (b >= 0); L.sync[0] = a; L.sync[1] = b; L.bwd = bwd; L.scalars = scalars; L.eval_stats = 0;
   return L;
 }
 
@@ -494,27 +598,26 @@
   extern __shared__ __align__(16) float dsm[];
   float* wbuf = dsm;
   float* xs = dsm + kWBuf;
+  float* bns = xs + kXS * kRC;
   __shared__ __align__(16) float w0s[kD * 20 + 64];
   __shared__ double shd[64];
-  __shared__ unsigned s_epoch;
+  __shared__ unsigned long long s_grid[2];
   const int tid = threadIdx.x, lane = tid & 31, warp = tid >> 5;
   if (tid == 0 && blockIdx.x == 0 && d.trace != nullptr) { unsigned long long t; asm volatile("mov.u64 %0, %%globaltimer;" : "=l"(t)); d.trace[31] = t; }
-  if (tid == 0) s_epoch = ld_relaxed_u32(d.bar + 32);
   for (int i = tid; i < kD * 20; i += kT2) w0s[i] = h.s_w0[i];
   if (tid < 20) { w0s[800 + tid] = h.s_b0[tid]; w0s[820 + tid] = h.s_w1[tid]; }
   if (tid == 0) w0s[840] = h.s_b1[0];
-  __syncthreads();
-  unsigned epoch = s_epoch;
-  int n_barrier = 0;
+  Grid G = grid_start(d, s_grid);
   const bool train = d.training != 0;
   const int T = d.T;
   const Rows R = my_rows(d.B);
   const int64_t tok0 = (int64_t)R.b0 * T, tok1 = (int64_t)R.b1 * T;
   auto sync_point = [&](const Leader& L, const Prefetch& pf) {
-    if (train) grid_barrier(h, d, epoch, L, n_barrier, wbuf, pf);
+    if (train) grid_sync(h, d, G, L, bns, wbuf, pf);
     else { __syncthreads(); copy_weights(wbuf, pf, tid, kT2); __syncthreads(); }
   };
-  if (!train) { Leader L = leader_of(-1, -1, 0, 0); L.eval_stats = 1; grid_barrier(h, d, epoch, L, n_barrier, wbuf, no_prefetch()); }
+  if (!train) { Leader L = leader_of(-1, -1, 0); L.eval_stats = 1; grid_sync(h, d, G, L, bns, wbuf, no_prefetch()); }
+  if (flat_mode(d) && blockIdx.x == 0) zero_copies(h.gsums[BN_T1], h.bn[BN_T1].C);
 
   if (train && blockIdx.x == 0) {
     const int G = d.B / PAMREC_GROUP;
@@ -580,11 +683,12 @@
         if (t != 0.0) atomicAdd(grp_fwd(h, BN_S0) + 2 * c + which, t);
       }
     }
-    sync_point(leader_of(BN_S0, -1, 0, 1, 1), Prefetch{h.e_w0, 5 * 4000, h.g_w0, 2 * 2560});
+    sync_point(leader_of(BN_S0, -1, 0, 1), Prefetch{h.e_w0, 5 * 4000, h.g_w0, 2 * 2560});
   }
   __syncthreads();
   {
     const BnSet& s0 = h.bn[BN_S0];
+    const float* st0 = bn_sh(bns, BN_S0);
     double s = 0.0, q = 0.0;
     for (int64_t tok = tok0 + tid; tok < tok1; tok += kT2) {
       const float* zr = h.z1 + tok * 20;
@@ -592,10 +696,10 @@
 #pragma unroll
       for (int i = 0; i < 5; ++i) {
         const float4 x = ld4(zr + 4 * i);
-        z = fmaf(bn_act(x.x, bn_c(s0, 4 * i)), w0s[820 + 4 * i], z);
-        z = fmaf(bn_act(x.y, bn_c(s0, 4 * i + 1)), w0s[820 + 4 * i + 1], z);
-        z = fmaf(bn_act(x.z, bn_c(s0, 4 * i + 2)), w0s[820 + 4 * i + 2], z);
-        z = fmaf(bn_act(x.w, bn_c(s0, 4 * i + 3)), w0s[820 + 4 * i + 3], z);
+        z = fmaf(bn_act(x.x, bn_c(s0, st0, 4 * i)), w0s[820 + 4 * i], z);
+        z = fmaf(bn_act(x.y, bn_c(s0, st0, 4 * i + 1)), w0s[820 + 4 * i + 1], z);
+        z = fmaf(bn_act(x.z, bn_c(s0, st0, 4 * i + 2)), w0s[820 + 4 * i + 2], z);
+        z = fmaf(bn_act(x.w, bn_c(s0, st0, 4 * i + 3)), w0s[820 + 4 * i + 3], z);
       }
       h.z2[tok] = z;
       s += (double)z; q += (double)z * (double)z;
@@ -604,11 +708,11 @@
       s = block_sum_d(s, shd); q = block_sum_d(q, shd);
       if (tid == 0 && (s != 0.0 || q != 0.0)) { atomicAdd(grp_fwd(h, BN_S1), s); atomicAdd(grp_fwd(h, BN_S1) + 1, q); }
     }
-    sync_point(leader_of(BN_S1, -1, 0, 1), no_prefetch());
+    sync_point(leader_of(BN_S1, -1, 0), no_prefetch());
   }
   __syncthreads();
   {
-    const BnC k1 = bn_c(h.bn[BN_S1], 0);
+    const BnC k1 = bn_c(h.bn[BN_S1], bn_sh(bns, BN_S1), 0);
     float* aws = xs;
     for (int b = R.b0 + warp; b < R.b1; b += kT2 / 32) {
       const int64_t base = (int64_t)b * T;
@@ -662,15 +766,15 @@
         else if (col < 628) add_sums(grp_fwd(h, BN_G0), col - 500, s[pass], q[pass]);
       }
     }
-    sync_point(leader_of(BN_E0, BN_G0, 0, 0), Prefetch{h.e_w1, 5 * 6400, h.g_w1, 2 * 320});
+    sync_point(leader_of(BN_E0, BN_G0, 0), Prefetch{h.e_w1, 5 * 6400, h.g_w1, 2 * 320});
   }
   {
     double s = 0.0, q = 0.0;
     for (int row0 = R.b0; row0 < R.b1; row0 += kRC) {
       const int nr = min(kRC, R.b1 - row0);
       __syncthreads();
-      stage_act(xs, 0, h.ze0, 500, 500, row0, nr, h.bn[BN_E0]);
-      stage_act(xs, 500, h.zg0, 128, 128, row0, nr, h.bn[BN_G0]);
+      stage_act(xs, 0, h.ze0, 500, 500, row0, nr, h.bn[BN_E0], bn_sh(bns, BN_E0));
+      stage_act(xs, 500, h.zg0, 128, 128, row0, nr, h.bn[BN_G0], bn_sh(bns, BN_G0));
       __syncthreads();
       const int col = tid;
       float acc[kRC];
@@ -690,7 +794,7 @@
       if (tid < 320) add_sums(grp_fwd(h, BN_E1), tid, s, q);
       else if (tid < 330) add_sums(grp_fwd(h, BN_G1), tid - 320, s, q);
     }
-    sync_point(leader_of(BN_E1, BN_G1, 0, 0), Prefetch{h.t_w0, 3 * 8400, nullptr, 0});
+    sync_point(leader_of(BN_E1, BN_G1, 0), Prefetch{h.t_w0, 3 * 8400, nullptr, 0});
   }
   {
     double s = 0.0, q = 0.0;
@@ -698,8 +802,8 @@
     for (int row0 = R.b0; row0 < R.b1; row0 += kRC) {
       const int nr = min(kRC, R.b1 - row0);
       __syncthreads();
-      stage_act(es, 0, h.ze1, 320, 320, row0, nr, h.bn[BN_E1]);
-      stage_act(es, 320, h.zg1, 10, 10, row0, nr, h.bn[BN_G1]);
+      stage_act(es, 0, h.ze1, 320, 320, row0, nr, h.bn[BN_E1], bn_sh(bns, BN_E1));
+      stage_act(es, 320, h.zg1, 10, 10, row0, nr, h.bn[BN_G1], bn_sh(bns, BN_G1));
       __syncthreads();
       if (tid < 168) {
         const int c = tid;
@@ -735,14 +839,14 @@
       }
     }
     if (train && tid < 300) add_sums(grp_fwd(h, BN_T0), tid, s, q);
-    sync_point(leader_of(BN_T0, -1, 0, 0), Prefetch{h.t_w1, 3 * 6400, nullptr, 0});
+    sync_point(leader_of(BN_T0, -1, 0), Prefetch{h.t_w1, 3 * 6400, nullptr, 0});
   }
   {
     double s = 0.0, q = 0.0;
     for (int row0 = R.b0; row0 < R.b1; row0 += kRC) {
       const int nr = min(kRC, R.b1 - row0);
       __syncthreads();
-      stage_act(xs, 0, h.zt0, 300, 300, row0, nr, h.bn[BN_T0]);
+      stage_act(xs, 0, h.zt0, 300, 300, row0, nr, h.bn[BN_T0], bn_sh(bns, BN_T0));
       __syncthreads();
       if (tid < 192) {
         const int g = tid / 64, n = tid % 64;
@@ -753,13 +857,13 @@
       }
     }
     if (train && tid < 192) add_sums(grp_fwd(h, BN_T1), tid, s, q);
-    sync_point(leader_of(BN_T1, -1, 0, 0), no_prefetch());
+    sync_point(leader_of(BN_T1, -1, 0), no_prefetch());
   }
   {
     for (int row0 = R.b0; row0 < R.b1; row0 += kRC) {
       const int nr = min(kRC, R.b1 - row0);
       __syncthreads();
-      stage_act(xs, 0, h.zt1, 192, 192, row0, nr, h.bn[BN_T1]);
+      stage_act(xs, 0, h.zt1, 192, 192, row0, nr, h.bn[BN_T1], bn_sh(bns, BN_T1));
       __syncthreads();
       if (tid < 3 * kRC) {
         const int g = tid / kRC, r = tid % kRC;
@@ -772,7 +876,7 @@
       }
     }
   }
-  if (tid == 0 && blockIdx.x == 0 && d.trace != nullptr) { unsigned long long t; asm volatile("mov.u64 %0, %%globaltimer;" : "=l"(t)); d.trace[30] = t; d.trace[29] = (unsigned long long)n_barrier; }
+  if (tid == 0 && blockIdx.x == 0 && d.trace != nullptr) { unsigned long long t; asm volatile("mov.u64 %0, %%globaltimer;" : "=l"(t)); d.trace[30] = t; d.trace[29] = (unsigned long long)G.n; }
   if (train) head2_transpose_weights(h);
 }
 
@@ -781,22 +885,20 @@
   float* wbuf = dsm;
   float* xs = dsm + kWBuf;
   float* aux = xs + kXS * kRC;
+  float* bns = aux + 4096;
   __shared__ double shd[64];
-  __shared__ unsigned s_epoch;
+  __shared__ unsigned long long s_grid[2];
   const int tid = threadIdx.x, lane = tid & 31, warp = tid >> 5;
   if (tid == 0 && blockIdx.x == 0 && d.trace != nullptr) { unsigned long long t; asm volatile("mov.u64 %0, %%globaltimer;" : "=l"(t)); d.trace[31] = t; }
-  if (tid == 0) s_epoch = ld_relaxed_u32(d.bar + 32);
-  __syncthreads();
-  unsigned epoch = s_epoch;
-  int n_barrier = 0;
+  Grid G = grid_start(d, s_grid);
+  if (flat_mode(d) && blockIdx.x == 0) zero_copies(h.gbsums[BN_S0], h.bn[BN_S0].C);
   const int T = d.T;
   const Rows R = my_rows(d.B);
   const int64_t tok0 = (int64_t)R.b0 * T, tok1 = (int64_t)R.b1 * T;
   const float* wT = h.wT;
 
   {
-    const int G = d.B / PAMREC_GROUP;
-    const int n_ndcg = (G + 3) / 4;
+    const int n_ndcg = (d.B / PAMREC_GROUP + 3) / 4;
     const int n_units = d.sm_group > 0 ? 2 * (d.B / d.sm_group) : 2 * d.B;
     const int n_rows = max((n_units + 31) / 32, 1);
     const int workers = max((int)gridDim.x - 1, 1), me = gridDim.x > 1 ? (int)blockIdx.x - 1 : 0;
@@ -804,7 +906,7 @@
       for (int i = me + workers * warp; i < n_ndcg + n_rows; i += workers * (kT2 / 32)) {
         if (i < n_ndcg) loss_ndcg_item(h, d, i); else loss_rows_item(h, d, i - n_ndcg);
       }
-    grid_barrier(h, d, epoch, leader_of(-1, -1, 1, 0), n_barrier, wbuf, Prefetch{wT + kWT_t1, 3 * 6400, nullptr, 0});
+    grid_sync(h, d, G, leader_of(-1, -1, 1), bns, wbuf, Prefetch{wT + kWT_t1, 3 * 6400, nullptr, 0});
   }
   {
     double s1 = 0.0, s2 = 0.0;
@@ -822,7 +924,7 @@
       }
       add_sums(grp_bwd(h, BN_T1), tid, s1, s2);
     }
-    grid_barrier(h, d, epoch, leader_of(BN_T1, -1, 1, 0), n_barrier, wbuf, no_prefetch());
+    grid_sync(h, d, G, leader_of(BN_T1, -1, 1), bns, wbuf, no_prefetch());
   }
   {
     double s1 = 0.0, s2 = 0.0;
@@ -830,7 +932,7 @@
     for (int row0 = R.b0; row0 < R.b1; row0 += kRC) {
       const int nr = min(kRC, R.b1 - row0);
       __syncthreads();
-      stage_dz(xs, 0, h.d_t1, h.zt1, 192, 192, row0, nr, h.bn[BN_T1], d.cntB);
+      stage_dz(xs, 0, h.d_t1, h.zt1, 192, 192, row0, nr, h.bn[BN_T1], bn_sh(bns, BN_T1));
       __syncthreads();
       if (tid < 300) {
         const int g = tid / 100, kk = tid % 100;
@@ -841,7 +943,7 @@
       }
     }
     if (tid < 300) add_sums(grp_bwd(h, BN_T0), tid, s1, s2);
-    grid_barrier(h, d, epoch, leader_of(BN_T0, -1, 1, 0), n_barrier, wbuf, Prefetch{wT + kWT_t0, 3 * 8400, nullptr, 0});
+    grid_sync(h, d, G, leader_of(BN_T0, -1, 1), bns, wbuf, Prefetch{wT + kWT_t0, 3 * 8400, nullptr, 0});
   }
   {
     double s1 = 0.0, s2 = 0.0;
@@ -852,9 +954,9 @@
     for (int row0 = R.b0; row0 < R.b1; row0 += kRC) {
       const int nr = min(kRC, R.b1 - row0);
       __syncthreads();
-      stage_dz(xs, 0, h.d_t0, h.zt0, 300, 300, row0, nr, h.bn[BN_T0], d.cntB);
-      stage_act(gt, 0, h.zg1, 10, 10, row0, nr, h.bn[BN_G1]);
-      stage_act(xs, 300, h.ze1, 320, 320, row0, nr, h.bn[BN_E1]);
+      stage_dz(xs, 0, h.d_t0, h.zt0, 300, 300, row0, nr, h.bn[BN_T0], bn_sh(bns, BN_T0));
+      stage_act(gt, 0, h.zg1, 10, 10, row0, nr, h.bn[BN_G1], h.bn[BN_G1].stat);
+      stage_act(xs, 300, h.ze1, 320, 320, row0, nr, h.bn[BN_E1], h.bn[BN_E1].stat);
       __syncthreads();
       if (tid < 168) {
         float acc[kRC];
@@ -900,7 +1002,7 @@
     }
     if (tid < 320) add_sums(grp_bwd(h, BN_E1), tid, s1, s2);
     else if (tid < 400) add_sums(grp_bwd(h, BN_G1), (tid - 320) >> 3, s1, s2);
-    grid_barrier(h, d, epoch, leader_of(BN_E1, BN_G1, 1, 0), n_barrier, wbuf, Prefetch{wT + kWT_e1, 5 * 6400 + 2 * 320, nullptr, 0});
+    grid_sync(h, d, G, leader_of(BN_E1, BN_G1, 1), bns, wbuf, Prefetch{wT + kWT_e1, 5 * 6400 + 2 * 320, nullptr, 0});
   }
   {
     double s1[2] = {0.0, 0.0}, s2[2] = {0.0, 0.0};
@@ -913,8 +1015,8 @@
     for (int row0 = R.b0; row0 < R.b1; row0 += kRC) {
       const int nr = min(kRC, R.b1 - row0);
       __syncthreads();
-      stage_dz(xs, 0, h.d_e1, h.ze1, 320, 320, row0, nr, h.bn[BN_E1], d.cntB);
-      stage_dz(xs, 320, h.d_g1, h.zg1, 10, 10, row0, nr, h.bn[BN_G1], d.cntB);
+      stage_dz(xs, 0, h.d_e1, h.ze1, 320, 320, row0, nr, h.bn[BN_E1], bn_sh(bns, BN_E1));
+      stage_dz(xs, 320, h.d_g1, h.zg1, 10, 10, row0, nr, h.bn[BN_G1], bn_sh(bns, BN_G1));
       __syncthreads();
 #pragma unroll
       for (int pass = 0; pass < 2; ++pass) {
@@ -939,7 +1041,7 @@
       if (col < 500) add_sums(grp_bwd(h, BN_E0), col, s1[pass], s2[pass]);
       else if (col < 628) add_sums(grp_bwd(h, BN_G0), col - 500, s1[pass], s2[pass]);
     }
-    grid_barrier(h, d, epoch, leader_of(BN_E0, BN_G0, 1, 0), n_barrier, wbuf, Prefetch{wT + kWT_x0, 628 * 40, nullptr, 0});
+    grid_sync(h, d, G, leader_of(BN_E0, BN_G0, 1), bns, wbuf, Prefetch{wT + kWT_x0, 628 * 40, nullptr, 0});
   }
   {
     const BnC k1 = bn_c(h.bn[BN_S1], 0);
@@ -949,8 +1051,8 @@
     for (int row0 = R.b0; row0 < R.b1; row0 += kRC) {
       const int nr = min(kRC, R.b1 - row0);
       __syncthreads();
-      stage_dz(xs, 0, h.d_e0, h.ze0, 500, 500, row0, nr, h.bn[BN_E0], d.cntB);
-      stage_dz(xs, 500, h.d_g0, h.zg0, 128, 128, row0, nr, h.bn[BN_G0], d.cntB);
+      stage_dz(xs, 0, h.d_e0, h.ze0, 500, 500, row0, nr, h.bn[BN_E0], bn_sh(bns, BN_E0));
+      stage_dz(xs, 500, h.d_g0, h.zg0, 128, 128, row0, nr, h.bn[BN_G0], bn_sh(bns, BN_G0));
       __syncthreads();
       if (tid < 480) {
         const int grp = tid / 40, c = tid % 40;
@@ -1009,7 +1111,7 @@
     }
     b1 = block_sum_d(b1, shd); b2 = block_sum_d(b2, shd);
     if (tid == 0 && (b1 != 0.0 || b2 != 0.0)) { atomicAdd(grp_bwd(h, BN_S1), b1); atomicAdd(grp_bwd(h, BN_S1) + 1, b2); }
-    grid_barrier(h, d, epoch, leader_of(BN_S1, -1, 1, 1), n_barrier, wbuf, no_prefetch());
+    grid_sync(h, d, G, leader_of(BN_S1, -1, 1), bns, wbuf, no_prefetch());
   }
   float* w0s = aux;
   float* w0t = aux + 800;
@@ -1019,7 +1121,7 @@
   for (int i = tid; i < 800; i += kT2) { const float v = h.s_w0[i]; w0s[i] = v; w0t[(i % 20) * 40 + i / 20] = v; }
   if (tid < 20) w1s[tid] = h.s_w1[tid];
   {
-    const BnB k1 = bn_b(h.bn[BN_S1], 0, d.cntN);
+    const BnB k1 = bn_b(h.bn[BN_S1], bn_sh(bns, BN_S1), 0);
     const int slot = tid / 20, j = tid % 20;
     double s1 = 0.0, s2 = 0.0, gw = 0.0, gb = 0.0;
     __syncthreads();
@@ -1050,15 +1152,15 @@
         else if (c == 0) atomicAdd(h.ds_b1, (float)t);
       }
     }
-    grid_barrier(h, d, epoch, leader_of(BN_S0, -1, 1, 1), n_barrier, wbuf, no_prefetch());
+    grid_sync(h, d, G, leader_of(BN_S0, -1, 1), bns, wbuf, no_prefetch());
   }
   {
     constexpr int kTB = 2 * kSlots;
-    const BnB k1 = bn_b(h.bn[BN_S1], 0, d.cntN);
+    const BnB k1 = bn_b(h.bn[BN_S1], bn_sh(bns, BN_S1), 0);
     const int slot = tid / 20, j = tid % 20;
     const int sl_h = tid / 10, kq = tid % 10;
     if (tid < 20) {
-      const BnB k = bn_b(h.bn[BN_S0], tid, d.cntN);
+      const BnB k = bn_b(h.bn[BN_S0], bn_sh(bns, BN_S0), tid);
       c0[6 * tid] = k.mean; c0[6 * tid + 1] = k.inv; c0[6 * tid + 2] = k.ga; c0[6 * tid + 3] = k.be; c0[6 * tid + 4] = k.s1n; c0[6 * tid + 5] = k.s2n;
     }
     float* Hs = xs;
@@ -1139,7 +1241,7 @@
       if (t != 0.0) atomicAdd(h.ds_b0 + tid, (float)t);
     }
   }
-  if (tid == 0 && blockIdx.x == 0 && d.trace != nullptr) { unsigned long long t; asm volatile("mov.u64 %0, %%globaltimer;" : "=l"(t)); d.trace[30] = t; d.trace[29] = (unsigned long long)n_barrier; }
+  if (tid == 0 && blockIdx.x == 0 && d.trace != nullptr) { unsigned long long t; asm volatile("mov.u64 %0, %%globaltimer;" : "=l"(t)); d.trace[30] = t; d.trace[29] = (unsigned long long)G.n; }
 }
 
 namespace {
@@ -1208,8 +1310,8 @@
   }
 }
 
-constexpr size_t kFwdSmem = (size_t)(kWBuf + kXS * kRC) * sizeof(float);
-constexpr size_t kBwdSmem = (size_t)(kWBuf + kXS * kRC + 4096) * sizeof(float);
+constexpr size_t kFwdSmem = (size_t)(kWBuf + kXS * kRC + 2 * kHead2BnTotal) * sizeof(float);
+constexpr size_t kBwdSmem = (size_t)(kWBuf + kXS * kRC + 4096 + 2 * kHead2BnTotal) * sizeof(float);
 int head2_grid() {
   int dev = 0, sms = 0, coop = 0, occ_f = 0, occ_b = 0;
   if (cudaGetDevice(&dev) != cudaSuccess) return -1;
```

Measured after the change: 1.428 million, median of 6. 1.03x the previous value.
